# VitorMPCastro/MessyerRaytracer

Hardware: AMD Instinct MI355X
Metric: Mrays/s (primary, closest-hit) (higher is better)
Workload: dtype f32

## Files before the change

__graft_entry__.py:

```python
import os
import sys

ROOT = os.path.dirname(os.path.abspath(__file__))
if ROOT not in sys.path:
    sys.path.insert(0, ROOT)


def build() -> None:
    from messyerraytracer_amd import build as b
    b.build_lib()
    b.build_host_test()
    b.build_host_cpu_test()
    b.build_host_tlas_test()
    b.build_policy_test()
    b.build_shadow_policy_test()
    b.build_reflection_policy_test()
    b.build_hemisphere_policy_test()
    b.build_bounce_policy_test()
    b.build_instance_math_test()
    b.build_build_rules_test()
    b.build_shade_data_test()
    b.build_light_data_test()
    b.build_path_data_test()
    b.build_texture_data_test()
    b.build_panorama_data_test()
    b.build_channel_data_test()
    b.build_lane_map_test()
    from oracle import pyoracle
    pyoracle.build(force=False)
    if os.path.isdir("/root/reference") and not pyoracle.ref_available():
        pyoracle.build(force=True)
    import messyerraytracer_amd
    from messyerraytracer_amd import capi
    L = capi.load()
    missing = [s for s in capi.SYMBOLS if not hasattr(L, s)]
    if missing:
        raise RuntimeError(f"libmrt_hip.so does not export {missing}")


def smoke() -> None:
    import numpy as np
    from messyerraytracer_amd import capi, synth
    from oracle import pyoracle as po

    ctx = capi.Context(0)
    for verts, (w, h), origin, fwd, fov in (
            (synth.cube(), (16, 12), (0, 0, 3), (0, 0, -1), 60.0),
            (synth.soup(2000, 0.4, 3), (128, 96), (0, 0, -12), (0, 0, 1), 50.0)):
        scene = capi.Scene(verts)
        scene.upload(ctx)
        cam = capi.camera_look(origin, fwd, w, h, fov)
        got = ctx.cast_grid(cam, w, h)
        osc = po.OracleScene(verts)
        rays = po.grid_rays(origin, fwd, w, h, fov)
        want = osc.trace(rays)
        assert (got["prim_id"] == want["prim_id"]).all(), "prim_id mismatch vs oracle"
        hit = want["prim_id"] >= 0
        assert np.array_equal(got["t"][hit], want["t"][hit]), "t mismatch vs oracle"
        assert hit.any() and (~hit).any()
    local, inst = synth.multi_mesh_instances(4, 500, 0.3, 5)
    ctx.upload_two_level_scene(local, inst)
    got = ctx.cast_grid(cam, w, h)
    want = po.OracleTwoLevelScene(local, inst).trace(rays)
    assert (got["prim_id"] == want["prim_id"]).all() and np.array_equal(got["t"], want["t"]), "two-level scene mismatch vs oracle"
    assert (want["prim_id"] >= 0).any()
    from messyerraytracer_amd import surface as S, types as T
    n = w * h
    mats = np.zeros(2, T.MATERIAL)
    mats["albedo"], mats["roughness"], mats["emission"], mats["emission_energy"] = 0.5, (0.02, 0.7), 1.0, (0.0, 2.0)
    shade = S.ShadeData(1500, mats, np.arange(1500) % 3)
    ctx.upload_shade_data(shade.n_tris, shade.materials, shade.material_ids)
    d_hits, d_rows = ctx.device_alloc(n * 32), ctx.device_alloc(n * 64)
    ctx.h2d(d_hits, got)
    ctx.resolve_grid_surfaces(cam, w, h, d_hits, d_rows)
    rows = np.zeros(n, T.SURFACE64)
    ctx.d2h(rows, d_rows)
    surf, _, _ = S.resolve(rays["direction"], got["normal"], got["prim_id"] != -1, got["prim_id"].view(np.uint32), got["bary_u"],
                           got["bary_v"], shade)
    assert np.array_equal(rows.view(np.uint32), surf.view(np.uint32)), "surface rows mismatch vs the restatement"
    from messyerraytracer_amd import channels as Ch
    d_normal, d_depth8 = ctx.device_alloc(n * 16), ctx.device_alloc(n * 4)
    ctx.shade_grid_channels(cam, w, h, d_hits, 0.125, 1.0, {Ch.NORMAL: d_normal}, {Ch.DEPTH: d_depth8})
    normal, depth8 = np.zeros((n, 4), np.float32), np.zeros((n, 4), np.uint8)
    ctx.d2h(normal, d_normal)
    ctx.d2h(depth8, d_depth8)
    want = Ch.shade_channels(rays["direction"], Ch.hit_position(rays["origin"], rays["direction"], got["t"]), got["normal"],
                             got["prim_id"] != -1, got["t"], got["prim_id"].view(np.uint32), got["bary_u"], got["bary_v"],
                             np.float32(0.125), np.float32(1.0), shade, None, (Ch.NORMAL, Ch.DEPTH))
    assert np.array_equal(normal.view(np.uint32), want[Ch.NORMAL].view(np.uint32)), "normal channel mismatch vs the restatement"
    assert np.array_equal(depth8, Ch.to_rgba8(want[Ch.DEPTH])), "depth bytes mismatch vs the restatement"
    ctx.device_free(d_normal)
    ctx.device_free(d_depth8)
    ctx.device_free(d_hits)
    ctx.device_free(d_rows)
    ctx.close()
    print("smoke ok")


if __name__ == "__main__":
    build()
    if len(sys.argv) > 1 and sys.argv[1] == "smoke":
        smoke()
```

messyerraytracer_amd/build.py:

```python
import concurrent.futures
import glob
import os
import shutil
import subprocess

HERE = os.path.dirname(os.path.abspath(__file__))
CSRC = os.path.join(HERE, "csrc")
LIB = os.path.join(HERE, "libmrt_hip.so")
OBJ = os.path.join(HERE, "_obj")

SOURCES = ["kernels.hip", "shade_kernels.hip", "prep_kernels.hip", "api.hip", "cast.hip", "schedule.hip", "launch_policy.cpp", "group.hip",
           "device_build.hip", "refit.hip", "tlas_device.hip", "surface.hip", "texture.hip", "lighting.hip", "path.hip", "panorama.hip", "channels.hip",
           "host/shade_data.cpp", "host/texture_data.cpp", "host/light_data.cpp", "host/path_data.cpp", "host/panorama_data.cpp", "host/channel_data.cpp", "host/scene_prep.cpp", "host/bvh_builder.cpp", "host/two_level_prep.cpp"]
FLAGS = ["--offload-arch=gfx950", "-O3", "-std=c++17", "-fPIC", "-ffp-contract=off", "-Wall",
         "-Wno-unused-result", "-Xarch_host", "-mfma"]

MIRROR = ["-O2", "-std=c++17", "-ffp-contract=off", "-Wall"]
POLICY = ["-O2", "-std=c++17", "-Wall"]
CPU = ["-x", "c++", "-O2", "-std=c++17", "-ffp-contract=off", "-Wall"]
LANE = ["-x", "c++", "-std=c++17", "-Wall"]
DRIVERS = {
    "host_mirror_test": (["host/host_mirror_test.cpp"], MIRROR, True),
    "host_cpu_test": (["host/host_cpu_test.cpp"], MIRROR, True),
    "host_tlas_test": (["host/host_tlas_test.cpp"], MIRROR, True),
    "launch_policy_test": (["host/launch_policy_test.cpp", "launch_policy.cpp"], POLICY, False),
    "shadow_policy_test": (["host/shadow_policy_test.cpp", "launch_policy.cpp"], POLICY, False),
    "reflection_policy_test": (["host/reflection_policy_test.cpp", "launch_policy.cpp"], POLICY, False),
    "hemisphere_policy_test": (["host/hemisphere_policy_test.cpp", "launch_policy.cpp"], POLICY, False),
    "bounce_policy_test": (["host/bounce_policy_test.cpp", "launch_policy.cpp"], POLICY, False),
    "instance_math_test": (["host/instance_math_test.cpp"], CPU, False),
    "build_rules_test": (["host/build_rules_test.cpp"], CPU, False),
    "build_rules_test_san": (["host/build_rules_test.cpp"], CPU[:2] + ["-O1", "-g", "-fno-omit-frame-pointer", "-std=c++17", "-ffp-contract=off", "-Wall",
                                                               "-fsanitize=address,undefined", "-fno-sanitize-recover=undefined"], False),
    "shade_data_test": (["host/shade_data_test.cpp", "host/shade_data.cpp"], CPU, False),
    "light_data_test": (["host/light_data_test.cpp", "host/light_data.cpp"], CPU, False),
    "path_data_test": (["host/path_data_test.cpp", "host/path_data.cpp"], CPU, False),
    "texture_data_test": (["host/texture_data_test.cpp", "host/texture_data.cpp"], CPU, False),
    "panorama_data_test": (["host/panorama_data_test.cpp", "host/panorama_data.cpp"], CPU, False),
    "channel_data_test": (["host/channel_data_test.cpp", "host/channel_data.cpp"], CPU, False),
    "lane_map_test": (["host/lane_map_test.cpp"], LANE + ["-O2"], False),
    "lane_map_test_san": (["host/lane_map_test.cpp"], LANE + ["-O1", "-g", "-fno-omit-frame-pointer", "-fsanitize=address,undefined",
                                                              "-fno-sanitize-recover=undefined"], False),
}


def _hipcc() -> str:
    for c in (shutil.which("hipcc"), "/opt/rocm/bin/hipcc"):
        if c and os.path.exists(c):
            return c
    raise RuntimeError("hipcc not found: libmrt_hip.so cannot be built")


def _run(cmd, what: str) -> str:
    r = subprocess.run(cmd, capture_output=True, text=True, cwd=CSRC)
    if r.returncode != 0:
        raise RuntimeError(what + " failed:\n" + " ".join(cmd) + "\n" + r.stdout + r.stderr)
    return r.stderr


def _stale(target: str, deps) -> bool:
    if deps is None or not os.path.exists(target):
        return True
    t = os.path.getmtime(target)
    return any(not os.path.exists(d) or os.path.getmtime(d) > t for d in list(deps) + [os.path.abspath(__file__)])


def _deps(dfile: str):
    if not os.path.exists(dfile):
        return None
    with open(dfile) as f:
        words = f.read().replace("\\\n", " ").split()
    return [os.path.join(CSRC, w) for w in words if not w.endswith(":")]


def define_set(env) -> list:
    return sorted((["-DMRT_WITH_QUAD"] if env.get("MRT_WITH_QUAD") == "1" else []) + env.get("MRT_EXTRA_DEFINES", "").split())


def defines_changed(stamp, defines) -> bool:
    return stamp is None or stamp.split() != sorted(defines)


def pool_size(n_sources: int, env, limit: int = 16) -> int:
    jobs = min(n_sources, limit)
    if env.get("MAX_JOBS", "").isdigit() and int(env["MAX_JOBS"]) > 0:
        jobs = min(jobs, int(env["MAX_JOBS"]))
    return max(jobs, 1)


def build_lib(force: bool = False, verbose: bool = False, lib: str = None, obj_dir: str = None, defines=None) -> str:
    lib, obj_dir = os.path.abspath(lib or LIB), os.path.abspath(obj_dir or OBJ)
    defines = define_set(os.environ) if defines is None else sorted(defines)
    stamp = os.path.join(obj_dir, "defines.txt")
    objs = [os.path.join(obj_dir, s.replace("/", "_") + ".o") for s in SOURCES]
    old = open(stamp).read() if os.path.exists(stamp) else None
    force = force or defines_changed(old, defines)
    all_deps = [_deps(o + ".d") for o in objs]
    if not force and not _stale(lib, None if None in all_deps else [d for ds in all_deps for d in ds]):
        return lib
    os.makedirs(obj_dir, exist_ok=True)
    if force and old is not None:
        os.remove(stamp)
    jobs = [(s, o) for s, o, ds in zip(SOURCES, objs, all_deps) if force or _stale(o, ds)]

    def compile_one(job):
        src, obj = job
        log = _run([_hipcc()] + FLAGS + defines + ["-MD", "-MF", obj + ".d", "-c", os.path.join(CSRC, src), "-o", obj], "hipcc")
        with open(obj + ".d") as f:
            text = f.read().replace(CSRC + os.sep, "")
        with open(obj + ".d", "w") as f:
            f.write(text)
        return log

    with concurrent.futures.ThreadPoolExecutor(max_workers=pool_size(len(SOURCES), os.environ)) as pool:
        logs = list(pool.map(compile_one, jobs))
    with open(stamp, "w") as f:
        f.write(" ".join(defines) + "\n")
    if jobs or _stale(lib, objs):
        logs.append(_run([_hipcc(), "--offload-arch=gfx950", "-shared", "-fPIC"] + objs + ["-o", lib, "-pthread"], "hipcc link"))
    if verbose:
        print("".join(logs))
    return lib


def build_driver(name: str, force: bool = False) -> str:
    srcs, flags, links = DRIVERS[name]
    srcs, exe = [os.path.join(CSRC, s) for s in srcs], os.path.join(HERE, name)
    headers = [h for pat in ("*.h", "*.inc", "host/*.h", "host/*.hpp", "../../include/*.h") for h in glob.glob(os.path.join(CSRC, pat))]
    if force or _stale(exe, srcs + headers + ([LIB] if links else [])):
        _run([_hipcc()] + flags + srcs + ["-o", exe] + (["-L" + HERE, "-lmrt_hip", "-Wl,-rpath," + HERE, "-pthread"] if links else []), name + " build")
    return exe


def _driver(name: str):
    def build(force: bool = False) -> str:
        return build_driver(name, force)
    build.__doc__ = "C++ test driver " + name + " (DRIVERS)."
    return build


build_host_test = _driver("host_mirror_test")
build_host_cpu_test = _driver("host_cpu_test")
build_host_tlas_test = _driver("host_tlas_test")
build_policy_test = _driver("launch_policy_test")
build_shadow_policy_test = _driver("shadow_policy_test")
build_reflection_policy_test = _driver("reflection_policy_test")
build_hemisphere_policy_test = _driver("hemisphere_policy_test")
build_bounce_policy_test = _driver("bounce_policy_test")
build_instance_math_test = _driver("instance_math_test")
build_shade_data_test = _driver("shade_data_test")
build_light_data_test = _driver("light_data_test")
build_path_data_test = _driver("path_data_test")
build_texture_data_test = _driver("texture_data_test")
build_panorama_data_test = _driver("panorama_data_test")
build_channel_data_test = _driver("channel_data_test")


def build_build_rules_test(force: bool = False, sanitize: bool = False) -> str:
    return build_driver("build_rules_test_san" if sanitize else "build_rules_test", force)


def build_lane_map_test(force: bool = False, sanitize: bool = False) -> str:
    return build_driver("lane_map_test_san" if sanitize else "lane_map_test", force)


if __name__ == "__main__":
    print(build_lib(force=True, verbose=True))
    for name in DRIVERS:
        if not name.endswith("_san"):
            print(build_driver(name, force=True))
```

messyerraytracer_amd/csrc/kernels.hip:

```cpp
#include <hip/hip_runtime.h>
#include <cfloat>
#include <cstdio>
#include <cstdlib>
#include <type_traits>
#include "mrt_internal.h"
#include "launch_policy.h"
#include "lane_map.h"

namespace mrt {

#include "device_common.h"
#include "dispatch.h"

#include "source_common.h"
#include "shadow_kernel.h"
#include "reflection_kernel.h"
#include "hemisphere_kernel.h"
#include "bounce_kernel.h"

template <bool ANY_HIT, bool COUNT>
__global__ __launch_bounds__(MRT_WG) void trace_lane_kernel(const TraceParams p)
{
	constexpr int SRC = SRC_CAST;
	const NoSource s{};
#include "lane_walk.inc"
}

#include "lane_persistent_kernel.h"
#include "packet_kernel.h"
#include "packet_asm_kernel.h"
#include "packet_rows_kernel.h"
#ifdef MRT_WITH_QUAD
#include "packet_quad_kernel.h"
#endif
#include "two_level_kernel.h"

template <class S, int SRC, bool ANY_HIT>
__global__ __launch_bounds__(MRT_WG) void trace_source_lane_kernel(const TraceParams p, const S s)
{
	constexpr bool COUNT = false;
#include "lane_walk.inc"
}
template <class S, int SRC, bool ANY_HIT>
__global__ __launch_bounds__(MRT_WG) void trace_source_two_level_kernel(const TraceParams p, const S s)
{
#include "two_level_walk.inc"
}
template <class S, int SRC, bool ANY_HIT, int WIDTH, bool TL>
__global__ __launch_bounds__(MRT_WG) MRT_PERSIST_ATTR void trace_source_persistent_kernel(const TraceParams p, const PersistParams q, const S s)
{
	constexpr bool COUNT = false;
#include "persistent_walk.inc"
}

bool quad_kernel_built()
{
#ifdef MRT_WITH_QUAD
	return true;
#else
	return false;
#endif
}
static thread_local char g_variant[96] = "";
const char *last_trace_variant() { return g_variant; }
#ifndef MRT_ROWS_WG_LARGE
#define MRT_ROWS_WG_LARGE MRT_WG
#endif

hipError_t launch_trace(const TraceParams &p_in, bool any_hit, bool count, hipStream_t stream)
{
	const TraceLaunch l = resolve_trace(p_in, any_hit, count, quad_kernel_built(), MRT_ROWS_WG_LARGE);
	if (l.error) return hipErrorInvalidValue;
	if (l.blocks == 0) return hipSuccess;
	TraceParams p = p_in;
	p.tile_group = l.tile_group;
	const TraceVariant &v = l.v;
	const Bool a{v.any_hit}, c{v.count};
	const auto go = [&](auto kernel) { hipLaunchKernelGGL(kernel, dim3(l.blocks), dim3(l.threads), l.lds, stream, p); };
	switch (v.kernel) {
		case TraceKernel::TWO_LEVEL_PACKET: dispatch([&](auto A) { go(trace_two_level_packet_kernel<A>); }, a); break;
		case TraceKernel::TWO_LEVEL: dispatch([&](auto A) { go(trace_two_level_kernel<A>); }, a); break;
#ifdef MRT_WITH_QUAD
		case TraceKernel::PACKET_QUAD: dispatch([&](auto C, auto A) { go(trace_packet_quad_kernel<A, C>); }, c, a); break;
#endif
		case TraceKernel::PACKET_ROWS:
			if (v.packets == 2u)
				dispatch([&](auto W, auto F, auto C, auto A) { go(trace_packet_rows_kernel<A, C, 2, W, F>); },
						Among<64, MRT_ROWS_WG_LARGE>{(int)v.wg}, Bool{v.cull}, c, a);
			else dispatch([&](auto C, auto A) { go(trace_packet_rows_kernel<A, C, 1, MRT_WG, false>); }, c, a);
			break;
		case TraceKernel::PACKET_ASM:
			dispatch([&](auto C, auto KPF, auto A) { if constexpr (!(C && KPF)) go(trace_packet_asm_kernel<A, C, KPF>); }, c, Bool{v.prefetch}, a);
			break;
		case TraceKernel::PACKET: dispatch([&](auto A, auto C) { go(trace_packet_kernel<A, C>); }, a, c); break;
		case TraceKernel::LANE: dispatch([&](auto A, auto C) { go(trace_lane_kernel<A, C>); }, a, c); break;
		default: return hipErrorInvalidValue;
	}
	format_variant(g_variant, sizeof(g_variant), v);
	return hipGetLastError();
}

static PersistParams persist_params(const TraceParams &p, unsigned long long *next_ray, uint32_t *overflow,
		uint32_t lds_depth, uint32_t refill, uint32_t leaf_wait, uint32_t blocks)
{
	PersistParams q;
	q.next_ray = next_ray; q.overflow = overflow; q.overflow_stride = blocks * MRT_WG;
	q.lds_depth = lds_depth; q.refill = refill; q.leaf_wait = leaf_wait ? leaf_wait : 1u;
	const uint64_t per_wave = p.count / ((uint64_t)blocks * (MRT_WG / MRT_WAVE)) / 32u;
	q.chunk = per_wave >= MRT_RAY_CHUNK ? MRT_RAY_CHUNK : (per_wave <= MRT_WAVE ? MRT_WAVE : (uint32_t)(per_wave & ~63ull));
	return q;
}

hipError_t launch_trace_persistent(const TraceParams &p, unsigned long long *next_ray, uint32_t *overflow,
		uint32_t lds_depth, uint32_t refill, uint32_t leaf_wait, uint32_t blocks, bool any_hit, bool count, hipStream_t stream)
{
	const TraceLaunch l = resolve_persistent(p, lds_depth, blocks, any_hit, count);
	if (l.blocks == 0) return hipSuccess;
	const PersistParams q = persist_params(p, next_ray, overflow, lds_depth, refill, leaf_wait, blocks);
	const TraceVariant &v = l.v;
	dispatch([&](auto TL, auto C, auto W, auto A) {
		if constexpr (!TL || (W != 4 && !C))
			hipLaunchKernelGGL((trace_lane_persistent_kernel<A, W, TL, C>), dim3(l.blocks), dim3(l.threads), l.lds, stream, p, q);
	}, Bool{v.two_level}, Bool{v.count}, Among<8, 4, 2>{v.width}, Bool{v.any_hit});
	format_variant(g_variant, sizeof(g_variant), v);
	return hipGetLastError();
}

template <class S>
hipError_t launch_source(const TraceParams &p, const void *params, int src, bool any_hit, unsigned long long *next_ray, uint32_t *overflow,
		uint32_t lds_depth, uint32_t refill, uint32_t leaf_wait, uint32_t blocks, hipStream_t stream)
{
	using F = SourceFamily<S>;
	const S &s = *static_cast<const S *>(params);
	const TraceLaunch l = resolve_source(p, lds_depth, blocks, any_hit);
	if (l.error) return hipErrorInvalidValue;
	if (l.blocks == 0) return hipSuccess;
	if ((src != F::ray32 && src != F::host && src != F::grid) || !(any_hit ? F::any_hit : F::nearest)) return hipErrorInvalidValue;
	const TraceVariant &v = l.v;
	const dim3 grid(l.blocks), wg(l.threads);
	const PersistParams q = blocks ? persist_params(p, next_ray, overflow, lds_depth, refill, leaf_wait, blocks) : PersistParams{};
	dispatch([&](auto A, auto SRC, auto TL, auto W) {
		if constexpr ((A ? F::any_hit : F::nearest) && (!TL || W != 4)) {
			if (v.kernel == TraceKernel::TWO_LEVEL) hipLaunchKernelGGL((trace_source_two_level_kernel<S, SRC, A>), grid, wg, l.lds, stream, p, s);
			else if (v.kernel == TraceKernel::LANE) hipLaunchKernelGGL((trace_source_lane_kernel<S, SRC, A>), grid, wg, l.lds, stream, p, s);
			else hipLaunchKernelGGL((trace_source_persistent_kernel<S, SRC, A, W, TL>), grid, wg, l.lds, stream, p, q, s);
		}
	}, Bool{any_hit}, Among<F::ray32, F::host, F::grid>{src}, Bool{v.two_level}, Among<8, 4, 2>{v.width});
	format_variant(g_variant, sizeof(g_variant), v, F::name, src, F::any_hit && F::nearest);
	return hipGetLastError();
}
template hipError_t launch_source<ShadowParams>(const TraceParams &, const void *, int, bool, unsigned long long *, uint32_t *, uint32_t, uint32_t, uint32_t, uint32_t, hipStream_t);
template hipError_t launch_source<ReflectParams>(const TraceParams &, const void *, int, bool, unsigned long long *, uint32_t *, uint32_t, uint32_t, uint32_t, uint32_t, hipStream_t);
template hipError_t launch_source<HemiParams>(const TraceParams &, const void *, int, bool, unsigned long long *, uint32_t *, uint32_t, uint32_t, uint32_t, uint32_t, hipStream_t);
template hipError_t launch_source<BounceParams>(const TraceParams &, const void *, int, bool, unsigned long long *, uint32_t *, uint32_t, uint32_t, uint32_t, uint32_t, hipStream_t);

}
```

messyerraytracer_amd/csrc/lane_map.h:

```cpp
#pragma once
#include <cstdint>

#if defined(__HIPCC__) || defined(__HIP__)
#define MRT_LM_HD __host__ __device__ __forceinline__
#else
#define MRT_LM_HD inline
#endif

namespace mrt {

struct TileGrid {
	uint32_t grid_w, rows;
	uint32_t tiles_x, tiles_y;
	uint32_t k;
	uint32_t order;
	uint32_t group;
	uint32_t quarter_all;
	const uint32_t *sched;
	uint32_t unit, sched_slots;
};

constexpr uint32_t kPieceTile = 20u, kPieceTile16 = 21u, kPieceNone = 0xFFu;
constexpr uint32_t kNextAnew = 0u, kNextSame = 1u, kNextRight = 2u, kNextRowMajor = 3u, kNextNone = 4u;
struct WaveTile {
	uint32_t tx, ty;
	uint32_t code;
};

MRT_LM_HD uint32_t tile_rows_of(uint32_t rows, uint32_t k) { return (rows + (64u >> k) - 1u) >> (6u - k); }

MRT_LM_HD bool sched_matches(uint64_t total, uint32_t unit, uint32_t n_units)
{
	if (n_units == 0u) return total == 0u;
	return (uint64_t)(n_units - 1u) * unit < total && total <= (uint64_t)n_units * unit;
}

template <class T>
MRT_LM_HD bool strip_tile(const TileGrid &g, T tile, uint32_t &tx, uint32_t &ty)
{
	const uint32_t tg = g.group ? g.group : 1u;
	uint32_t m = (g.tiles_x + 128u) >> 8;
	if (m == 0u) m = 1u;
	const uint32_t S = g.tiles_x / (8u * m);
	if (S == 0u || S * 8u * m != g.tiles_x || S % tg != 0u) return false;
	const T wg = tile / tg;
	const uint32_t x = (uint32_t)wg & 7u;
	const T j = (wg >> 3) * tg + (tile - wg * tg);
	const T per_strip = (T)S * g.tiles_y;
	const T q = j / per_strip;
	const uint32_t sl = (uint32_t)q, r = (uint32_t)(j - q * per_strip);
	ty = r / S;
	tx = (sl * 8u + x) * S + r % S;
	return true;
}

template <class T>
MRT_LM_HD WaveTile wave_tile_t(const TileGrid &g, T group)
{
	WaveTile w; w.tx = 0u; w.ty = 0u; w.code = kPieceNone;
	const T total = (T)g.tiles_x * g.tiles_y;
	T tile = group;
	uint32_t piece = kPieceTile, next = kNextAnew;
	bool plus1 = false;
	if (g.quarter_all == 2u) {
		piece = (uint32_t)tile & 15u; tile >>= 4;
		if (tile >= total) return w;
		if (piece < 15u) next = kNextSame;
	} else if (g.quarter_all) {
		piece = 16u + ((uint32_t)tile & 3u); tile >>= 2;
		if (tile >= total) return w;
		if (piece < 19u) next = kNextSame;
	} else if (g.sched != nullptr) {
		const T slot = g.unit == 1u ? tile : (g.unit == 2u ? tile >> 1 : tile / g.unit);
		const uint32_t rem = (uint32_t)(tile - slot * g.unit);
		if (slot >= g.sched_slots) return w;
		const uint32_t e = g.sched[slot], what = e >> 28, id = e & 0x0FFFFFFFu;
		if (what == 0u) { tile = (T)id * g.unit + rem; plus1 = rem + 1u < g.unit; }
		else {
			if (rem != 0u) return w;
			tile = id;
			if (what >= 2u) piece = what - 2u < 4u ? 16u + (what - 2u) : kPieceTile16;
			if (g.unit > 1u) next = kNextNone;
		}
	} else plus1 = true;
	const bool even = ((uint32_t)tile & 1u) == 0u;
	if (g.order == 1u && (g.tiles_x & 15u) == 0u && (g.tiles_y & 15u) == 0u) {
		const uint32_t st = (uint32_t)(tile >> 8), in = (uint32_t)tile & 255u;
		uint32_t mx = in & 0x55u, my = (in >> 1) & 0x55u;
		mx = (mx | (mx >> 1)) & 0x33u; mx = (mx | (mx >> 2)) & 0x0Fu;
		my = (my | (my >> 1)) & 0x33u; my = (my | (my >> 2)) & 0x0Fu;
		const uint32_t sx = g.tiles_x >> 4, sty = st / sx;
		w.tx = ((st - sty * sx) << 4) + mx; w.ty = (sty << 4) + my;
		if (plus1 && even) next = kNextRight;
	} else if (g.order == 2u && (g.tiles_x & 31u) == 0u && (g.tiles_y & 31u) == 0u) {
		const uint32_t st = (uint32_t)(tile >> 10), in = (uint32_t)tile & 1023u;
		uint32_t mx = in & 0x155u, my = (in >> 1) & 0x155u;
		mx = (mx | (mx >> 1)) & 0x133u; mx = (mx | (mx >> 2)) & 0x10Fu; mx = (mx | (mx >> 4)) & 0x1Fu;
		my = (my | (my >> 1)) & 0x133u; my = (my | (my >> 2)) & 0x10Fu; my = (my | (my >> 4)) & 0x1Fu;
		const uint32_t sx = g.tiles_x >> 5, sty = st / sx;
		w.tx = ((st - sty * sx) << 5) + mx; w.ty = (sty << 5) + my;
		if (plus1 && even) next = kNextRight;
	} else if (g.order == 3u && strip_tile<T>(g, tile, w.tx, w.ty)) {
		if (plus1 && even && g.group != 0u && (g.group & 1u) == 0u) next = kNextRight;
	} else {
		const T y = tile / g.tiles_x;
		w.tx = (uint32_t)(tile - y * g.tiles_x); w.ty = (uint32_t)y;
		if (plus1) next = kNextRowMajor;
	}
	w.code = piece | next << 8;
	return w;
}

MRT_LM_HD WaveTile wave_tile(const TileGrid &g, uint64_t group)
{
	const bool narrow = (group >> 32) == 0u && (((uint64_t)g.tiles_x * g.tiles_y) >> 32) == 0u && (g.sched == nullptr || g.unit <= 16u);
	return narrow ? wave_tile_t<uint32_t>(g, (uint32_t)group) : wave_tile_t<uint64_t>(g, group);
}

MRT_LM_HD WaveTile wave_tile_next(const TileGrid &g, const WaveTile &a, uint64_t group)
{
	WaveTile b = a;
	const uint32_t piece = a.code & 0xFFu, next = piece == kPieceNone ? kNextAnew : a.code >> 8;
	b.code = piece | kNextAnew << 8;
	if (next == kNextSame) { b.code += 1u; return b; }
	if (next == kNextNone) { b.code = kPieceNone; return b; }
	if (next == kNextRight) { b.tx = a.tx + 1u; return b; }
	if (next == kNextRowMajor) {
		b.tx = a.tx + 1u;
		if (b.tx == g.tiles_x) { b.tx = 0u; b.ty = a.ty + 1u; }
		return b;
	}
	return wave_tile(g, group + 1u);
}

MRT_LM_HD bool tile_lane(const TileGrid &g, const WaveTile &w, uint32_t l, uint64_t &ray_idx, uint32_t &px, uint32_t &py)
{
	const uint32_t piece = w.code & 0xFFu;
	if (piece == kPieceNone) return false;
	if (piece < 16u) {
		if (l >= 4u) return false;
		px = (w.tx << 3) + ((piece & 3u) << 1) + (l & 1u);
		py = (w.ty << 3) + ((piece >> 2) << 1) + (l >> 1);
	} else if (piece < kPieceTile) {
		if (l >= 16u) return false;
		px = (w.tx << 3) + ((piece & 1u) << 2) + (l & 3u);
		py = (w.ty << 3) + (((piece >> 1) & 1u) << 2) + (l >> 2);
	} else {
		if (piece == kPieceTile16 && l >= 16u) return false;
		px = (w.tx << g.k) + (l & ((1u << g.k) - 1u));
		py = (w.ty << (6u - g.k)) + (l >> g.k);
	}
	if (px >= g.grid_w || py >= g.rows) return false;
	ray_idx = (uint64_t)py * g.grid_w + px;
	return true;
}

MRT_LM_HD bool linear_lane(uint64_t group, uint32_t l, uint32_t sparse_lanes, uint64_t count, uint64_t &entry)
{
	if (sparse_lanes) { if (l >= sparse_lanes) return false; entry = group * sparse_lanes + l; }
	else entry = (group << 6) + l;
	return entry < count;
}

}
```

messyerraytracer_amd/csrc/mrt_internal.h:

```cpp
#pragma once
#include <cstdint>
#include "../../include/mrt_hip.h"

static_assert(sizeof(mrt_ray32) == 32, "GPURayPacked must be 32 bytes (src/api/gpu_types.h:70)");
static_assert(sizeof(mrt_hit32) == 32, "GPUIntersectionPacked must be 32 bytes (src/api/gpu_types.h:93)");
static_assert(sizeof(mrt_tri64) == 64, "GPUTrianglePacked must be 64 bytes (src/api/gpu_types.h:51)");
static_assert(sizeof(mrt_bvh_node32) == 32, "GPUBVHNodePacked must be 32 bytes (src/api/gpu_types.h:127)");
static_assert(sizeof(mrt_bvh_node_wide64) == 64, "GPUBVHNodeWide must be 64 bytes (src/gpu/gpu_structs.h:47)");
static_assert(sizeof(mrt_host_ray60) == 60, "Ray must be 60 bytes (src/core/ray.h:25-51, precision=single)");
static_assert(sizeof(mrt_host_hit44) == 44, "Intersection must be 44 bytes (src/core/intersection.h:16-40)");
static_assert(sizeof(mrt_host_tri80) == 80, "Triangle must be 80 bytes (src/core/triangle.h:22-39)");
static_assert(sizeof(mrt_light) == 32, "mrt_light must be 32 bytes");

namespace mrt {

struct alignas(16) DevNode {
	float lmin[3]; uint32_t left_ref;
	float lmax[3]; uint32_t right_ref;
	float rmin[3]; uint32_t left_count;
	float rmax[3]; uint32_t right_count;
};
static_assert(sizeof(DevNode) == 64, "DevNode must be 64 bytes");

struct alignas(16) TriHot {
	float v0[3]; uint32_t id;
	float e1[3]; uint32_t layers;
	float e2[3]; uint32_t flags;
};
static_assert(sizeof(TriHot) == 48, "TriHot must be 48 bytes");
struct alignas(16) TriCold { float normal[3]; uint32_t pad; };

struct alignas(16) Dev4Node {
	float box[4][6];
	uint32_t ref[4];
	uint32_t n_children, pad[3];
};
static_assert(sizeof(Dev4Node) == 128, "Dev4Node must be 128 bytes");

struct alignas(16) Dev8Node {
	float org[3];
	uint8_t exp[3];
	uint8_t n_children;
	uint8_t qlo[3][8];
	uint8_t qhi[3][8];
	uint32_t ref[8];
	uint32_t pad[8];
};
static_assert(sizeof(Dev8Node) == 128, "Dev8Node must be 128 bytes");

constexpr int kCntRays = 0, kCntTris = 1, kCntNodes = 2, kCntHits = 3, kCntMaxStack = 4, kCntDeadPops = 5;
constexpr int kCntWaveNodeFetch = 6;
constexpr int kCntWaveTriFetch = 7;
constexpr int kCntLeafBoxChecks = 8;
constexpr int kCntFetchWaitCycles = 9, kCntWaveCycles = 10, kCntWaves = 11;
constexpr int kNumCounters = 16;
constexpr int kAutoGridOff = kNumCounters;
constexpr int kDetectScratchOff = kAutoGridOff + 8;
constexpr int kNextRayOff = kDetectScratchOff + 1026;
constexpr int kCounterWords = kNextRayOff + 128;

constexpr uint32_t kWaveSlots = 8192u;

constexpr uint32_t kSentinel = 0x7FFFFFFFu;
constexpr uint32_t kLeafBit = 0x80000000u;
constexpr uint32_t kLastInLeaf = 1u;

enum InFmt : uint32_t { IN_RAY32 = 0, IN_HOST60 = 1, IN_GRID = 2 };
enum OutFmt : uint32_t { OUT_HIT32 = 0, OUT_HOST44 = 1, OUT_BOOL8 = 2, OUT_TOKEN4 = 3, OUT_TOKEN8 = 4 };
enum LaneMap : uint32_t { MAP_LINEAR = 0, MAP_TILE8X8 = 1, MAP_AUTO = 2 };

struct DevInstance;
struct TraceParams {
	const DevNode *nodes;
	const Dev4Node *nodes4;
	const Dev8Node *nodes8;
	const float *leaf_box;
	const DevInstance *instances;
	const TriHot *tri_hot;
	const TriCold *tri_cold;
	const void *row_array;
	const void *row_array4;
	uint32_t rows_wg;
	uint32_t rows_cull;
	float scene_abs_max;
	uint32_t tri_unit_base4;
	const void *rays;
	void *hits;
	const uint32_t *perm;
	unsigned long long *counters;
	const uint32_t *auto_grid;
	const uint32_t *skip_flag;
	uint32_t skip_when;
	uint64_t count;
	uint32_t query_mask;
	uint32_t in_fmt, out_fmt, lane_map;
	uint32_t grid_w, grid_h, y0, rows;
	uint32_t tiles_x;
	uint32_t tile_w_log2;
	uint32_t tile_order;
	uint32_t tile_group;
	const uint32_t *tile_sched;
	uint32_t *tile_cost;
	uint32_t tile_unit, n_units;
	const uint32_t *sched_hdr;
	uint32_t n_slots_max;
	uint32_t quarter_all;
	uint32_t sparse_lanes;
	uint32_t kernel;
	uint32_t stack_depth;
	uint32_t xcd_swizzle;
	uint32_t n_tris;
	uint32_t n_instances;
	uint32_t n_nodes;
	uint32_t count_mode;
	uint32_t extra_lds;
	mrt_camera cam;
};

enum RaySrc : int { SRC_CAST = 0, SRC_SHADOW_RAY32 = 1, SRC_SHADOW_HOST44 = 2, SRC_SHADOW_GRID = 3,
	SRC_REFLECT_RAY32 = 4, SRC_REFLECT_HOST = 5, SRC_REFLECT_GRID = 6,
	SRC_HEMI_RAY32 = 7, SRC_HEMI_HOST = 8, SRC_HEMI_GRID = 9,
	SRC_BOUNCE_RAY32 = 10, SRC_BOUNCE_HOST = 11, SRC_BOUNCE_GRID = 12 };
constexpr bool shadow_source(int src) { return src >= SRC_SHADOW_RAY32 && src <= SRC_SHADOW_GRID; }
constexpr bool reflection_source(int src) { return src >= SRC_REFLECT_RAY32 && src <= SRC_REFLECT_GRID; }
constexpr bool hemisphere_source(int src) { return src >= SRC_HEMI_RAY32 && src <= SRC_HEMI_GRID; }
constexpr bool bounce_source(int src) { return src >= SRC_BOUNCE_RAY32 && src <= SRC_BOUNCE_GRID; }
constexpr bool lit_output(int src, bool any_hit) { return shadow_source(src) || (hemisphere_source(src) && any_hit); }
enum ShadowKind : uint32_t { SHADOW_OFF = 0, SHADOW_DIRECTIONAL = 1, SHADOW_POINT = 2 };
struct ShadowLight { uint32_t kind; float v[3]; };
struct ShadowParams {
	const void *records;
	uint64_t pixels;
	ShadowLight light[MRT_MAX_LIGHTS];
};

struct ReflectParams {
	const void *records;
	const uint8_t *select;
	void *out_rays;
	float max_distance;
};

constexpr uint32_t kPcgMul = 747796405u, kPcgInc = 2891336453u;
struct HemiJump { uint32_t a, c; };
struct HemiParams {
	const void *records;
	const uint8_t *select;
	void *out_rays;
	uint64_t pixels;
	uint32_t seed_add;
	float t_max;
	HemiJump jump[MRT_MAX_HEMISPHERE_SAMPLES];
};

struct BounceParams {
	const void *records;
	const uint8_t *select;
	const float *surface;
	void *out_rays;
	uint8_t *out_lobe;
	uint32_t seed_add;
	float t_max;
	float metallic, roughness;
	HemiJump jump;
};

enum SurfaceSrc : int { SURF_RAY32 = 0, SURF_HOST = 1, SURF_GRID = 2 };
struct SurfaceParams {
	const void *records;
	const void *shade_rows;
	const void *materials;
	uint32_t n_tris, n_materials, present;
	void *out_rows;
	float *out_bounce;
	void *out_hits;
};

struct ChannelParams {
	const void *records;
	const void *shade_rows;
	const void *materials;
	uint32_t n_tris, n_materials, present;
	uint32_t mask;
	float inv_depth_range, inv_pos_range;
	float *rgba[MRT_CHANNEL_COUNT];
	uint8_t *rgba8[MRT_CHANNEL_COUNT];
};
constexpr uint32_t CHANNELS_ROW = (1u << MRT_CHANNEL_NORMAL) | (1u << MRT_CHANNEL_ALBEDO) | (1u << MRT_CHANNEL_UV) | (1u << MRT_CHANNEL_FRESNEL);
constexpr uint32_t CHANNELS_MATERIAL = (1u << MRT_CHANNEL_NORMAL) | (1u << MRT_CHANNEL_ALBEDO);

template <class S> struct SourceFamily;
template <> struct SourceFamily<ShadowParams> {
	static constexpr int ray32 = SRC_SHADOW_RAY32, host = SRC_SHADOW_HOST44, grid = SRC_SHADOW_GRID;
	static constexpr bool any_hit = true, nearest = false;
	static constexpr const char *name = "shadow";
};
template <> struct SourceFamily<ReflectParams> {
	static constexpr int ray32 = SRC_REFLECT_RAY32, host = SRC_REFLECT_HOST, grid = SRC_REFLECT_GRID;
	static constexpr bool any_hit = false, nearest = true;
	static constexpr const char *name = "reflection";
};
template <> struct SourceFamily<HemiParams> {
	static constexpr int ray32 = SRC_HEMI_RAY32, host = SRC_HEMI_HOST, grid = SRC_HEMI_GRID;
	static constexpr bool any_hit = true, nearest = true;
	static constexpr const char *name = "hemisphere";
};
template <> struct SourceFamily<BounceParams> {
	static constexpr int ray32 = SRC_BOUNCE_RAY32, host = SRC_BOUNCE_HOST, grid = SRC_BOUNCE_GRID;
	static constexpr bool any_hit = false, nearest = true;
	static constexpr const char *name = "bounce";
};

struct DeviceSceneHost {
	DevNode *nodes = nullptr; uint32_t n_nodes = 0;
	Dev4Node *nodes4 = nullptr; uint32_t n_nodes4 = 0;
	uint32_t stack4 = 0;
	bool want8 = false;
	Dev8Node *nodes8 = nullptr; uint32_t n_nodes8 = 0; uint32_t stack8 = 0;
	float *leaf_box = nullptr;
	float bounds_lo[3] = {0, 0, 0}, bounds_hi[3] = {0, 0, 0};
	TriHot *hot = nullptr; TriCold *cold = nullptr; uint32_t n_tris = 0;
	uint32_t depth = 0;
};
int prepare_scene(const mrt_tri64 *tris, uint32_t n_tris, const mrt_bvh_node32 *nodes, uint32_t used_nodes,
		const uint32_t *prim_idx, DeviceSceneHost *out, char *err, size_t err_len);

struct DeviceBuildResult {
	DevNode *nodes = nullptr; TriHot *hot = nullptr; TriCold *cold = nullptr;
	Dev4Node *nodes4 = nullptr;
	Dev8Node *nodes8 = nullptr;
	float *leaf_box = nullptr;
	uint32_t n_nodes = 0, n_tris = 0, depth = 0, stack4 = 0, stack8 = 0;
	float bounds_lo[3] = {0, 0, 0}, bounds_hi[3] = {0, 0, 0};
	uint32_t *slot_src = nullptr;
	const float *boxes_in = nullptr;
};
struct BuildArena { void *ptr = nullptr; size_t cap = 0; uint32_t *pinned = nullptr; };
int device_build_lbvh(const mrt_tri64 *d_tris, uint32_t n, bool want4, bool want8, bool safe_handoff, int form, BuildArena *arena, void *stream,
		DeviceBuildResult *out, char *err, size_t err_len);

constexpr uint32_t kAsmNodeLimit = 1u << 26;
constexpr uint32_t kInstanceReturn = 0x7FFFFFFEu;
using ::MRT_KERNEL_TWO_LEVEL; using ::MRT_KERNEL_TWO_LEVEL_PACKET; using ::MRT_KERNEL_TWO_LEVEL_PERSISTENT;
using ::MRT_KERNEL_TWO_LEVEL_PERSISTENT8;
struct alignas(16) DevInstance {
	float inv[12];
	float basis[9];
	uint32_t root;
	uint32_t id_base;
	uint32_t layers;
	uint32_t flags;
	uint32_t index;
	uint32_t root8;
	uint32_t pad[5];
};
static_assert(sizeof(DevInstance) == 128, "DevInstance must be 128 bytes");

struct TwoLevelBlas { uint32_t first_tri, n_tris, root, depth; float lo[3], hi[3]; uint32_t root8, stack8, n_nodes; };
struct TwoLevelHost {
	DevNode *nodes = nullptr; uint32_t n_nodes = 0, tlas_cap = 0, n_tlas_nodes = 0;
	TriHot *hot = nullptr; TriCold *cold = nullptr; uint32_t n_tris = 0;
	DevInstance *inst = nullptr; uint32_t n_inst = 0;
	TwoLevelBlas *blas = nullptr; uint32_t n_blas = 0;
	uint32_t *inst_blas = nullptr;
	uint32_t depth = 0;
	Dev8Node *nodes8 = nullptr; uint32_t n_nodes8 = 0; float *leaf_box = nullptr;
	bool wide8 = false;
	uint32_t depth8 = 0;
	uint64_t flat_tris = 0;
};
void free_two_level(TwoLevelHost *h);
int prepare_two_level(const float *verts9, uint32_t n_mesh_tris, const mrt_instance *instances, uint32_t n_instances,
		uint32_t n_threads, bool build_blas, TwoLevelHost *out, char *err, size_t err_len);

int refit_two_level(TwoLevelHost *h, const mrt_instance *instances, uint32_t n_instances, char *err, size_t err_len);
int check_two_level_refit(const TwoLevelHost *h, const mrt_instance *instances, uint32_t n_instances, uint32_t n_mesh_tris,
		char *err, size_t err_len);

}
```

messyerraytracer_amd/csrc/packet_rows_kernel.h:

```cpp
#pragma once

#define RA_LMINX "s20"
#define RA_LMINY "s21"
#define RA_LMINZ "s22"
#define RA_LREF "s23"
#define RA_LMAXX "s24"
#define RA_LMAXY "s25"
#define RA_LMAXZ "s26"
#define RA_RREF "s27"
#define RA_RMINX "s28"
#define RA_RMINY "s29"
#define RA_RMINZ "s30"
#define RA_RMAXX "s32"
#define RA_RMAXY "s33"
#define RA_RMAXZ "s34"
#define RA_MASK "s[60:61]"
#define RA_MASKLO "s60"
#define RA_MASKHI "s61"
#define RA_V0X "s20"
#define RA_V0Y "s21"
#define RA_V0Z "s22"
#define RA_ID "s23"
#define RA_E1X "s24"
#define RA_E1Y "s25"
#define RA_E1Z "s26"
#define RA_LAYERS "s27"
#define RA_E2X "s28"
#define RA_E2Y "s29"
#define RA_E2Z "s30"
#define RA_FLAGS "s31"

#define MRT_NEAR_0(RS, AX, SIDE) RS##_##SIDE##MIN##AX
#define MRT_NEAR_1(RS, AX, SIDE) RS##_##SIDE##MAX##AX
#define MRT_FAR_0(RS, AX, SIDE) RS##_##SIDE##MAX##AX
#define MRT_FAR_1(RS, AX, SIDE) RS##_##SIDE##MIN##AX

#define MRT_OP(NAME, P) "%[" NAME P "]"

#define MRT_ROWS_SLAB(P, RS, BX, BY, BZ)                                                                             \
	"v_fma_f32 v50, " MRT_NEAR_##BX(RS, X, L) ", " MRT_OP("ix", P) ", " MRT_OP("nrx", P) "\n"                        \
	"v_fma_f32 v51, " MRT_NEAR_##BY(RS, Y, L) ", " MRT_OP("iy", P) ", " MRT_OP("nry", P) "\n"                        \
	"v_fma_f32 v52, " MRT_NEAR_##BZ(RS, Z, L) ", " MRT_OP("iz", P) ", " MRT_OP("nrz", P) "\n"                        \
	"v_fma_f32 v53, " MRT_FAR_##BX(RS, X, L) ", " MRT_OP("ix", P) ", " MRT_OP("nrx", P) "\n"                         \
	"v_fma_f32 v54, " MRT_FAR_##BY(RS, Y, L) ", " MRT_OP("iy", P) ", " MRT_OP("nry", P) "\n"                         \
	"v_fma_f32 v55, " MRT_FAR_##BZ(RS, Z, L) ", " MRT_OP("iz", P) ", " MRT_OP("nrz", P) "\n"                         \
	"v_max_f32 v52, v52, " MRT_OP("tmin", P) "\n"                                                                   \
	"v_fma_f32 v56, " MRT_NEAR_##BX(RS, X, R) ", " MRT_OP("ix", P) ", " MRT_OP("nrx", P) "\n"                        \
	"v_min_f32 v55, v55, " MRT_OP("lim", P) "\n"                                                                    \
	"v_fma_f32 v57, " MRT_NEAR_##BY(RS, Y, R) ", " MRT_OP("iy", P) ", " MRT_OP("nry", P) "\n"                        \
	"v_max3_f32 v50, v50, v51, v52\n"                                                               \
	"v_fma_f32 v51, " MRT_NEAR_##BZ(RS, Z, R) ", " MRT_OP("iz", P) ", " MRT_OP("nrz", P) "\n"                        \
	"v_min3_f32 v53, v53, v54, v55\n"                                                               \
	"v_fma_f32 v52, " MRT_FAR_##BX(RS, X, R) ", " MRT_OP("ix", P) ", " MRT_OP("nrx", P) "\n"                         \
	"v_fma_f32 v54, " MRT_FAR_##BY(RS, Y, R) ", " MRT_OP("iy", P) ", " MRT_OP("nry", P) "\n"                         \
	"v_fma_f32 v55, " MRT_FAR_##BZ(RS, Z, R) ", " MRT_OP("iz", P) ", " MRT_OP("nrz", P) "\n"                         \
	"v_max_f32 v51, v51, " MRT_OP("tmin", P) "\n"                                                                   \
	"v_min_f32 v55, v55, " MRT_OP("lim", P) "\n"                                                                    \
	"v_max3_f32 v56, v56, v57, v51\n"                                                               \
	"v_min3_f32 v52, v52, v54, v55\n"

#define MRT_ROWS_NODE_STEP(P, RS, POPBIT, CNT_P, BX, BY, BZ)                                                                 \
	MRT_ROWS_SLAB(P, RS, BX, BY, BZ)                                                                                \
	"v_cmp_le_f32 vcc, v50, v53\n"                                             \
	"v_cmp_le_f32_e64 s[54:55], v56, v52\n"                                    \
	"s_cbranch_vccz L_" P "lmiss_%=\n"                                                                              \
	"s_cmp_eq_u64 s[54:55], 0\n"                                                                                    \
	"s_cbranch_scc1 L_" P "onlyl_%=\n"                                                                              \
	"v_cmp_lt_f32_e64 s[56:57], v50, v56\n"     \
	"s_bitcmp1_b32 s56, 0\n"                                                                                        \
	"s_cselect_b32 s53, " RS##_RREF ", " RS##_LREF "\n"                                                    \
	"s_cselect_b32 " MRT_OP("cur", P) ", " RS##_LREF ", " RS##_RREF "\n"                                   \
	"s_cselect_b64 s[58:59], s[54:55], vcc\n"                                   \
	"s_cselect_b64 " RS##_MASK ", vcc, s[54:55]\n"                               \
	"v_mov_b32 v51, s53\n"                                                                                          \
	"v_mov_b32 v52, s58\n"                                                                                          \
	"v_mov_b32 v53, s59\n"                                                                                          \
	"ds_write_b32 " MRT_OP("sp", P) ", v51\n"                                                                       \
	"ds_write_b64 " MRT_OP("sp", P) ", v[52:53] offset:8\n"                                                         \
	"v_add_u32 " MRT_OP("sp", P) ", 16, " MRT_OP("sp", P) "\n"                                                      \
	CNT_P                                                                                                           \
	"v_lshlrev_b32 v54, 6, v51\n"             \
	"global_load_dword v60, v54, %[rows]\n"   \
	"s_branch L_" P "done_%=\n"                                                                                     \
	"L_" P "onlyl_%=:\n"                                                                                            \
	"s_mov_b32 " MRT_OP("cur", P) ", " RS##_LREF "\n"                                                                \
	"s_mov_b64 " RS##_MASK ", vcc\n"                                                                                 \
	"s_branch L_" P "done_%=\n"                                                                                     \
	"L_" P "lmiss_%=:\n"                                                                                            \
	"s_cmp_eq_u64 s[54:55], 0\n"                                                                                    \
	"s_cbranch_scc1 L_" P "npop_%=\n"                                                                               \
	"s_mov_b32 " MRT_OP("cur", P) ", " RS##_RREF "\n"                                                                \
	"s_mov_b64 " RS##_MASK ", s[54:55]\n"                                                                            \
	"s_branch L_" P "done_%=\n"                                                                                     \
	"L_" P "npop_%=:\n"                                                                                             \
	"s_or_b32 %[ev], %[ev], " POPBIT "\n"

#define MRT_ROWS_TRI_TEST(P, RS, OWNMASK, CUROP, ANYHIT_CODE)                                                        \
	"s_and_b32 s52, " RS##_LAYERS ", %[qmask]\n"                    \
	"s_cbranch_scc0 L_" P "tnext_%=\n"                                                                              \
	"v_mul_f32 v50, " RS##_E2Y ", " MRT_OP("dz", P) "\n"                                                             \
	"v_mul_f32 v51, " RS##_E2Z ", " MRT_OP("dx", P) "\n"                                                             \
	"v_mul_f32 v52, " RS##_E2X ", " MRT_OP("dy", P) "\n"                                                             \
	"v_fma_f32 v50, " MRT_OP("dy", P) ", " RS##_E2Z ", -v50\n"                            \
	"v_fma_f32 v51, " MRT_OP("dz", P) ", " RS##_E2X ", -v51\n"                            \
	"v_fma_f32 v52, " MRT_OP("dx", P) ", " RS##_E2Y ", -v52\n"                            \
	"v_mul_f32 v53, " RS##_E1Z ", v52\n"                                                                             \
	"v_fma_f32 v53, " RS##_E1Y ", v51, v53\n"                                                                        \
	"v_fma_f32 v53, " RS##_E1X ", v50, v53\n"                                                     \
	"v_cmp_nlt_f32_e64 s[54:55], |v53|, %[eps]\n"                                              \
	"s_and_b64 s[54:55], s[54:55], " OWNMASK "\n"                       \
	"s_cbranch_scc0 L_" P "tnext_%=\n"                                                                              \
	"v_div_scale_f32 v54, s[56:57], v53, v53, 1.0\n"                   \
	"v_rcp_f32 v55, v54\n"                                                                                          \
	"v_div_scale_f32 v56, vcc, 1.0, v53, 1.0\n"                                                                     \
	"v_subrev_f32 v59, " RS##_V0X ", " MRT_OP("ox", P) "\n"       \
	"v_fma_f32 v57, -v54, v55, 1.0\n"                                                                               \
	"v_fma_f32 v55, v57, v55, v55\n"                                                                                \
	"v_mul_f32 v57, v56, v55\n"                                                                                     \
	"v_fma_f32 v58, -v54, v57, v56\n"                                                                               \
	"v_fma_f32 v57, v58, v55, v57\n"                                                                                \
	"v_fma_f32 v54, -v54, v57, v56\n"                                                                               \
	"v_div_fmas_f32 v54, v54, v55, v57\n"                                                                           \
	"v_div_fixup_f32 v54, v54, v53, 1.0\n"                                                       \
	"v_subrev_f32 v55, " RS##_V0Y ", " MRT_OP("oy", P) "\n"                                                 \
	"v_subrev_f32 v56, " RS##_V0Z ", " MRT_OP("oz", P) "\n"                                                 \
	"v_mul_f32 v58, v56, v52\n"                                                                                     \
	"v_fma_f32 v58, v55, v51, v58\n"                                                                                \
	"v_fma_f32 v58, v59, v50, v58\n"                                                                                \
	"v_mul_f32 v58, v58, v54\n"                                                    \
	"v_cmp_nlt_f32_e64 s[56:57], v58, 0\n"                                                            \
	"v_cmp_ngt_f32_e64 s[58:59], v58, 1.0\n"                                                          \
	"s_and_b64 s[54:55], s[54:55], s[56:57]\n"                                                                      \
	"s_and_b64 s[54:55], s[54:55], s[58:59]\n"                                                                      \
	"s_cbranch_scc0 L_" P "tnext_%=\n"                                                                              \
	"v_mul_f32 v50, " RS##_E1Y ", v56\n"                                                                             \
	"v_mul_f32 v51, " RS##_E1Z ", v59\n"                                                                             \
	"v_mul_f32 v52, " RS##_E1X ", v55\n"                                                                             \
	"v_fma_f32 v50, v55, " RS##_E1Z ", -v50\n"                                          \
	"v_fma_f32 v51, v56, " RS##_E1X ", -v51\n"                                          \
	"v_fma_f32 v52, v59, " RS##_E1Y ", -v52\n"                                          \
	"v_mul_f32 v59, " MRT_OP("dz", P) ", v52\n"                                                                     \
	"v_fma_f32 v59, " MRT_OP("dy", P) ", v51, v59\n"                                                                \
	"v_fma_f32 v59, " MRT_OP("dx", P) ", v50, v59\n"                                                                \
	"v_mul_f32 v59, v59, v54\n"                                                     \
	"v_add_f32 v55, v58, v59\n"                                                                          \
	"v_cmp_nlt_f32_e64 s[56:57], v59, 0\n"                                                            \
	"v_cmp_ngt_f32_e64 s[58:59], v55, 1.0\n"                                                      \
	"s_and_b64 s[54:55], s[54:55], s[56:57]\n"                                                                      \
	"s_and_b64 s[54:55], s[54:55], s[58:59]\n"                                                                      \
	"s_cbranch_scc0 L_" P "tnext_%=\n"                                                                              \
	"v_mul_f32 v55, " RS##_E2Z ", v52\n"                                                                             \
	"v_fma_f32 v55, " RS##_E2Y ", v51, v55\n"                                                                        \
	"v_fma_f32 v55, " RS##_E2X ", v50, v55\n"                                                                        \
	"v_mul_f32 v55, v55, v54\n"                                                    \
	                          \
	"v_cmp_nlt_f32_e64 s[56:57], v55, " MRT_OP("tmin", P) "\n"                                                      \
	"v_cmp_lt_f32_e64 s[58:59], v55, " MRT_OP("lim", P) "\n"                                                        \
	"v_cmp_eq_f32_e64 s[64:65], v55, " MRT_OP("lim", P) "\n"                                                        \
	"v_cmp_ne_u32_e64 s[66:67], " MRT_OP("bs", P) ", -1\n"                                                          \
	"v_cmp_gt_u32_e64 vcc, " MRT_OP("bi", P) ", " RS##_ID "\n"                                     \
	"s_and_b64 s[64:65], s[64:65], s[66:67]\n"                                                                      \
	"s_and_b64 s[64:65], s[64:65], vcc\n"                                                                           \
	"s_or_b64 s[58:59], s[58:59], s[64:65]\n"                                                                       \
	"s_and_b64 s[54:55], s[54:55], s[56:57]\n"                                                                      \
	"s_and_b64 s[54:55], s[54:55], s[58:59]\n"                                    \
	"s_cbranch_scc0 L_" P "tnext_%=\n"                                                                              \
	"s_and_b32 s52, " CUROP ", 0x7fffffff\n"                                                \
	"v_mov_b32 v50, s52\n"                                                                                          \
	"v_mov_b32 v51, " RS##_ID "\n"                                                                                   \
	"v_cndmask_b32_e64 " MRT_OP("bt", P) ", " MRT_OP("bt", P) ", v55, s[54:55]\n"                                   \
	"v_cndmask_b32_e64 " MRT_OP("bu", P) ", " MRT_OP("bu", P) ", v58, s[54:55]\n"                                   \
	"v_cndmask_b32_e64 " MRT_OP("bv", P) ", " MRT_OP("bv", P) ", v59, s[54:55]\n"                                   \
	"v_cndmask_b32_e64 " MRT_OP("bs", P) ", " MRT_OP("bs", P) ", v50, s[54:55]\n"                                   \
	"v_cndmask_b32_e64 " MRT_OP("bi", P) ", " MRT_OP("bi", P) ", v51, s[54:55]\n"                                   \
	ANYHIT_CODE                                                                                                     \
	"L_" P "tnext_%=:\n"

#define MRT_ROWS_TRI_STEP(P, RS, POPBIT, CNT_T, ANYHIT_CODE)                                                         \
	CNT_T                                                                                                           \
	MRT_ROWS_TRI_TEST(P, RS, RS##_MASK, MRT_OP("cur", P), ANYHIT_CODE)                                              \
	"s_bitcmp1_b32 " RS##_FLAGS ", 0\n"                                          \
	"s_cbranch_scc1 L_" P "tpop_%=\n"                                                                               \
	"s_add_u32 " MRT_OP("cur", P) ", " MRT_OP("cur", P) ", 1\n"                                                     \
	"s_branch L_" P "done_%=\n"                                                                                     \
	"L_" P "tpop_%=:\n"                                                                                             \
	"s_or_b32 %[ev], %[ev], " POPBIT "\n"

#define MRT_ROWS_NEAREST(P) \
	"v_cndmask_b32_e64 " MRT_OP("lim", P) ", " MRT_OP("lim", P) ", v55, s[54:55]\n"
#define MRT_ROWS_ANYHIT(P, DONEBIT) \
	"v_cndmask_b32_e64 " MRT_OP("lim", P) ", " MRT_OP("lim", P) ", %[vneg], s[54:55]\n"                             \
	"v_cmp_neq_f32_e64 s[56:57], " MRT_OP("lim", P) ", %[vneg]\n"                                                   \
	"s_cmp_lg_u64 s[56:57], 0\n"                                                                                    \
	"s_cbranch_scc1 L_" P "tnext_%=\n"                                                                              \
	"s_mov_b32 " MRT_OP("cur", P) ", 0x7fffffff\n"                                                                  \
	"s_or_b32 %[ev], %[ev], " DONEBIT "\n"                                                                          \
	"s_branch L_" P "done_%=\n"

#define MRT_ROWS_STEP(P, RS, POPBIT, CNT_N, CNT_T, CNT_P, ANYHIT_CODE, BX, BY, BZ)                                            \
	"s_bitcmp1_b32 " MRT_OP("cur", P) ", 31\n"                                                                      \
	"s_cbranch_scc1 L_" P "tri_%=\n"                                                                                \
	CNT_N                                                                                                           \
	MRT_ROWS_NODE_STEP(P, RS, POPBIT, CNT_P, BX, BY, BZ)                                                             \
	"s_branch L_" P "done_%=\n"                                                                                     \
	"L_" P "tri_%=:\n"                                                                                              \
	MRT_ROWS_TRI_STEP(P, RS, POPBIT, CNT_T, ANYHIT_CODE)                                                             \
	"L_" P "done_%=:\n"

#define MRT_ROWS_POP_ISSUE(P, POPBITNO, V0123)                                                                      \
	"s_bitcmp1_b32 %[ev], " POPBITNO "\n"                                                                           \
	"s_cbranch_scc0 L_" P "pi_%=\n"                                                                                 \
	"v_add_u32 " MRT_OP("sp", P) ", -16, " MRT_OP("sp", P) "\n"                                                     \
	"ds_read_b128 " V0123 ", " MRT_OP("sp", P) "\n"                                                                 \
	"L_" P "pi_%=:\n"
#define MRT_ROWS_POP_TAKE(P, RS, POPBITNO, V0, V2, V3)                                                               \
	"s_bitcmp1_b32 %[ev], " POPBITNO "\n"                                                                           \
	"s_cbranch_scc0 L_" P "pt_%=\n"                                                                                 \
	"v_readfirstlane_b32 " MRT_OP("cur", P) ", " V0 "\n"                                                            \
	"v_readfirstlane_b32 " RS##_MASKLO ", " V2 "\n"                                                                  \
	"v_readfirstlane_b32 " RS##_MASKHI ", " V3 "\n"                                                                  \
	"L_" P "pt_%=:\n"

#define MRT_ROWS_CLOBBERS                                                                                             \
	"vcc", "scc", "s20", "s21", "s22", "s23", "s24", "s25", "s26", "s27", "s28", "s29", "s30", "s31", "s32", "s33", \
	"s34", "s35", "s36", "s37", "s38", "s39", "s40", "s41", "s42", "s43", "s44", "s45", "s46", "s47", "s48", "s49", \
	"s50", "s51", "s52", "s53", "s54", "s55", "s56", "s57", "s58", "s59", "s60", "s61", "s62", "s63", "s64", "s65", \
	"s66", "s67", "v50", "v51", "v52", "v53", "v54", "v55", "v56", "v57", "v58", "v59", "v60"

#define MRT_ROWS_OUT(P, S)                                                                                            \
	[cur##P] "+s"(S.cur), [sp##P] "+v"(S.sp), [lim##P] "+v"(S.lim), [bt##P] "+v"(S.bt), [bu##P] "+v"(S.bu),         \
	[bv##P] "+v"(S.bv), [bs##P] "+v"(S.bs), [bi##P] "+v"(S.bi), [mask##P] "+s"(S.mask)
#define MRT_ROWS_IN(P, S)                                                                                             \
	[ox##P] "v"(S.ox), [oy##P] "v"(S.oy), [oz##P] "v"(S.oz), [dx##P] "v"(S.dx), [dy##P] "v"(S.dy), [dz##P] "v"(S.dz), \
	[tmin##P] "v"(S.tmin), [ix##P] "v"(S.ix), [iy##P] "v"(S.iy), [iz##P] "v"(S.iz), [nrx##P] "v"(S.nrx),            \
	[nry##P] "v"(S.nry), [nrz##P] "v"(S.nrz)

struct PacketRegs {
	float ox, oy, oz, dx, dy, dz, tmin;
	float ix, iy, iz, nrx, nry, nrz;
	float lim;
	float bt, bu, bv;
	uint32_t bs, bi;
	uint32_t sp;
	uint32_t cur;
	unsigned long long mask;
};

#define MRT_ROWS_LOOP1(CNT_N, CNT_T, CNT_P, T_PRE, T_POST, ANYHIT_CODE, BX, BY, BZ)                                          \
	asm volatile(                                                                                                   \
		"s_mov_b64 s[60:61], %[maskA]\n"                                                                            \
		"L_loop_%=:\n"                                                                                              \
		"s_lshl_b32 s52, %[curA], 6\n"                                                                              \
		T_PRE                                                                                                       \
		"s_load_dwordx16 s[20:35], %[rows], s52\n"                                                                  \
		"s_waitcnt lgkmcnt(0)\n"                                                                                    \
		T_POST                                                                                                      \
		MRT_ROWS_STEP("A", RA, "1", CNT_N, CNT_T, CNT_P, ANYHIT_CODE, BX, BY, BZ)                                   \
		"s_cmp_eq_u32 %[ev], 0\n"                                                                                   \
		"s_cbranch_scc1 L_loop_%=\n"                                                                                \
		MRT_ROWS_POP_ISSUE("A", "0", "v[50:53]")                                                                    \
		"s_waitcnt lgkmcnt(0)\n"                                                                                    \
		MRT_ROWS_POP_TAKE("A", RA, "0", "v50", "v52", "v53")                                                        \
		"s_mov_b32 %[ev], 0\n"                                                                                      \
		"s_cmp_lg_u32 %[curA], 0x7fffffff\n"                                                                        \
		"s_cbranch_scc1 L_loop_%=\n"                                                                                \
		"s_waitcnt vmcnt(0)\n"                    \
		"s_mov_b64 %[maskA], s[60:61]\n"                                                                            \
		: MRT_ROWS_OUT(A, a), [ev] "+s"(ev), [cntn] "+s"(cnt_n), [cntt] "+s"(cnt_t), [cntw] "+s"(cnt_w), [cntp] "+s"(sp_max) \
		: MRT_ROWS_IN(A, a), [rows] "s"(rows), [qmask] "s"(qmask), [eps] "s"(eps), [vneg] "v"(vneg)                 \
		: MRT_ROWS_CLOBBERS)

#define MRT_ROWSW_GROUP_SLAB(P, OWN, LM, RM, BX, BY, BZ)                                                              \
	"s_cmp_eq_u64 " OWN ", 0\n"                                                                                     \
	"s_cbranch_scc1 L_" P "skip_%=\n"                             \
	MRT_ROWS_SLAB(P, RA, BX, BY, BZ)                                                                                \
	"v_cmp_le_f32_e64 " LM ", v50, v53\n"                                                                           \
	"v_cmp_le_f32_e64 " RM ", v56, v52\n"                                                                           \
	"L_" P "sdone_%=:\n"
#define MRT_ROWSW_GROUP_SKIP(P, LM, RM)                                                                               \
	"L_" P "skip_%=:\n"                                                                                             \
	"s_mov_b64 " LM ", 0\n"                                                                                         \
	"s_mov_b64 " RM ", 0\n"                                                                                         \
	"s_branch L_" P "sdone_%=\n"

#define MRT_ROWSW_ANYHIT(P) \
	"v_cndmask_b32_e64 " MRT_OP("lim", P) ", " MRT_OP("lim", P) ", %[vneg], s[54:55]\n"
#define MRT_ROWSW_ANYDONE                                                                                             \
	"v_cmp_neq_f32_e64 s[56:57], %[limA], %[vneg]\n"                                                                \
	"v_cmp_neq_f32_e64 s[58:59], %[limB], %[vneg]\n"                                                                \
	"s_or_b64 s[56:57], s[56:57], s[58:59]\n"                                                                       \
	"s_cbranch_scc1 L_goon_%=\n"                                                                                    \
	"s_mov_b32 %[curA], 0x7fffffff\n"                                                                               \
	"s_branch L_exit_%=\n"                                                                                          \
	"L_goon_%=:\n"

#ifndef MRT_ROWS_KPREFETCH
#define MRT_ROWS_KPREFETCH 1
#endif
#if MRT_ROWS_KPREFETCH
#define MRT_ROWSW_KPREFETCH                                                                                           \
	"s_lshl_b32 s48, " RA_LREF ", 6\n"                                                                               \
	"s_lshl_b32 s49, " RA_RREF ", 6\n"                                                                               \
	"s_load_dword s64, %[rows], s48\n"                                                                              \
	"s_load_dword s65, %[rows], s49\n"
#define MRT_ROWSW_FARPREFETCH ""
#else
#define MRT_ROWSW_KPREFETCH ""
#define MRT_ROWSW_FARPREFETCH                                                                                         \
	"v_lshlrev_b32 v55, 6, v54\n"                                       \
	"global_load_dword v60, v55, %[rows]\n"
#endif

#define MRT_ROWS_LOOPW(CNT_N, CNT_T, CNT_P, ANYA, ANYB, ANYDONE, BX, BY, BZ)                                                 \
	asm volatile(                                                                                                   \
		"s_mov_b64 s[60:61], %[maskA]\n"                                                                            \
		"s_mov_b64 s[62:63], %[maskB]\n"                                                                            \
		"L_loop_%=:\n"                                                                                              \
		"s_lshl_b32 s52, %[curA], 6\n"                                                                              \
		"s_load_dwordx16 s[20:35], %[rows], s52\n"                                                                  \
		"s_waitcnt lgkmcnt(0)\n"                                                                                    \
		"s_bitcmp1_b32 %[curA], 31\n"                                                                               \
		"s_cbranch_scc1 L_tri_%=\n"                                                                                 \
		CNT_N                                                                                                       \
		MRT_ROWSW_KPREFETCH                                                                                         \
		MRT_ROWSW_GROUP_SLAB("A", "s[60:61]", "s[36:37]", "s[38:39]", BX, BY, BZ)                                   \
		MRT_ROWSW_GROUP_SLAB("B", "s[62:63]", "s[40:41]", "s[42:43]", BX, BY, BZ)                                   \
		"s_or_b64 s[44:45], s[36:37], s[40:41]\n"                     \
		"s_cbranch_scc0 L_lmiss_%=\n"                                                                               \
		"s_or_b64 vcc, s[38:39], s[42:43]\n"                                              \
		"s_cbranch_scc0 L_onlyl_%=\n"                                                                               \
		      \
		"v_cmp_lt_f32_e64 s[46:47], v50, v56\n"                                           \
		"s_bitcmp1_b32 s46, 0\n"                                                                                    \
		"s_cselect_b32 s53, " RA_RREF ", " RA_LREF "\n"                                                   \
		"s_cselect_b32 %[curA], " RA_LREF ", " RA_RREF "\n"                                               \
		"s_cselect_b64 s[50:51], s[38:39], s[36:37]\n"                 \
		"s_cselect_b64 s[58:59], s[42:43], s[40:41]\n"                                                              \
		"s_cselect_b64 s[60:61], s[36:37], s[38:39]\n"                                        \
		"s_cselect_b64 s[62:63], s[40:41], s[42:43]\n"                                                              \
		"v_mov_b32 v50, s50\n"                                                                                      \
		"v_mov_b32 v51, s51\n"                                                                                      \
		"v_mov_b32 v52, s58\n"                                                                                      \
		"v_mov_b32 v53, s59\n"                                                                                      \
		"v_mov_b32 v54, s53\n"                                                                                      \
		"ds_write_b128 %[spA], v[50:53]\n"                                                                          \
		"ds_write_b32 %[spA], v54 offset:16\n"                                                                      \
		"v_add_u32 %[spA], 32, %[spA]\n"                                                                            \
		CNT_P                                                                                                       \
		MRT_ROWSW_FARPREFETCH                                                                                       \
		"s_branch L_loop_%=\n"                                                                                      \
		"L_onlyl_%=:\n"                                                                                             \
		"s_mov_b32 %[curA], " RA_LREF "\n"                                                                          \
		"s_mov_b64 s[60:61], s[36:37]\n"                                                                            \
		"s_mov_b64 s[62:63], s[40:41]\n"                                                                            \
		"s_branch L_loop_%=\n"                                                                                      \
		"L_lmiss_%=:\n"                                                                                             \
		"s_or_b64 vcc, s[38:39], s[42:43]\n"                                                                        \
		"s_cbranch_scc0 L_pop_%=\n"                                                                                 \
		"s_mov_b32 %[curA], " RA_RREF "\n"                                                                          \
		"s_mov_b64 s[60:61], s[38:39]\n"                                                                            \
		"s_mov_b64 s[62:63], s[42:43]\n"                                                                            \
		"s_branch L_loop_%=\n"                                                                                      \
		"L_tri_%=:\n"                                                                                               \
		CNT_T                                                                                                       \
		"s_cmp_eq_u64 s[60:61], 0\n"                                                                                \
		"s_cbranch_scc1 L_Atnext_%=\n"                                                                              \
		MRT_ROWS_TRI_TEST("A", RA, "s[60:61]", "%[curA]", ANYA)                                                     \
		"s_cmp_eq_u64 s[62:63], 0\n"                                                                                \
		"s_cbranch_scc1 L_Btnext_%=\n"                                                                              \
		MRT_ROWS_TRI_TEST("B", RA, "s[62:63]", "%[curA]", ANYB)                                                     \
		ANYDONE                                                                                                     \
		"s_bitcmp1_b32 " RA_FLAGS ", 0\n"                                       \
		"s_cbranch_scc1 L_pop_%=\n"                                                                                 \
		"s_add_u32 %[curA], %[curA], 1\n"                                                                           \
		"s_branch L_loop_%=\n"                                                                                      \
		"L_pop_%=:\n"                                                                                               \
		"v_add_u32 %[spA], -32, %[spA]\n"                                                                           \
		"ds_read_b128 v[50:53], %[spA]\n"                                                                           \
		"ds_read_b32 v54, %[spA] offset:16\n"                                                                       \
		"s_waitcnt lgkmcnt(0)\n"                                                                                    \
		"v_readfirstlane_b32 %[curA], v54\n"                                                                        \
		"v_readfirstlane_b32 s60, v50\n"                                                                            \
		"v_readfirstlane_b32 s61, v51\n"                                                                            \
		"v_readfirstlane_b32 s62, v52\n"                                                                            \
		"v_readfirstlane_b32 s63, v53\n"                                                                            \
		"s_cmp_lg_u32 %[curA], 0x7fffffff\n"                                                                        \
		"s_cbranch_scc1 L_loop_%=\n"                                                                                \
		"s_branch L_exit_%=\n"                                                                                      \
		MRT_ROWSW_GROUP_SKIP("A", "s[36:37]", "s[38:39]")                                                           \
		MRT_ROWSW_GROUP_SKIP("B", "s[40:41]", "s[42:43]")                                                           \
		"L_exit_%=:\n"                                                                                              \
		"s_waitcnt vmcnt(0)\n"                    \
		"s_mov_b64 %[maskA], s[60:61]\n"                                                                            \
		"s_mov_b64 %[maskB], s[62:63]\n"                                                                            \
		: MRT_ROWS_OUT(A, a), [limB] "+v"(b.lim), [btB] "+v"(b.bt), [buB] "+v"(b.bu), [bvB] "+v"(b.bv),             \
		  [bsB] "+v"(b.bs), [biB] "+v"(b.bi), [maskB] "+s"(b.mask), [cntn] "+s"(cnt_n), [cntt] "+s"(cnt_t), [cntp] "+s"(sp_max) \
		: MRT_ROWS_IN(A, a), MRT_ROWS_IN(B, b), [rows] "s"(rows), [qmask] "s"(qmask), [eps] "s"(eps), [vneg] "v"(vneg) \
		: MRT_ROWS_CLOBBERS)


#define MRT_ROWS_SLAB1(P, RS, SIDE, TE, BX, BY, BZ, MASK)                                                             \
	"v_fma_f32 v51, " MRT_NEAR_##BX(RS, X, SIDE) ", " MRT_OP("ix", P) ", " MRT_OP("nrx", P) "\n"                      \
	"v_fma_f32 v52, " MRT_NEAR_##BY(RS, Y, SIDE) ", " MRT_OP("iy", P) ", " MRT_OP("nry", P) "\n"                      \
	"v_fma_f32 v53, " MRT_NEAR_##BZ(RS, Z, SIDE) ", " MRT_OP("iz", P) ", " MRT_OP("nrz", P) "\n"                      \
	"v_fma_f32 v54, " MRT_FAR_##BX(RS, X, SIDE) ", " MRT_OP("ix", P) ", " MRT_OP("nrx", P) "\n"                       \
	"v_fma_f32 v55, " MRT_FAR_##BY(RS, Y, SIDE) ", " MRT_OP("iy", P) ", " MRT_OP("nry", P) "\n"                       \
	"v_fma_f32 v57, " MRT_FAR_##BZ(RS, Z, SIDE) ", " MRT_OP("iz", P) ", " MRT_OP("nrz", P) "\n"                       \
	"v_max_f32 v53, v53, " MRT_OP("tmin", P) "\n"                                                                   \
	"v_min_f32 v57, v57, " MRT_OP("lim", P) "\n"                                                                    \
	"v_max3_f32 " TE ", v51, v52, v53\n"                                                                            \
	"v_min3_f32 v54, v54, v55, v57\n"                                                                               \
	"v_cmp_le_f32_e64 " MASK ", " TE ", v54\n"

#define MRT_ROWSC_CHILD(SIDE, TE, CULLBITS, MA, MB, BX, BY, BZ)                                                       \
	"s_and_b32 s48, s44, " CULLBITS "\n"                                 \
	"s_cbranch_scc1 L_cull" #SIDE "_%=\n"                                                                           \
	"s_cmp_eq_u64 s[60:61], 0\n"                                                                                    \
	"s_cbranch_scc1 L_" #SIDE "A0_%=\n"                                                                             \
	MRT_ROWS_SLAB1("A", RA, SIDE, TE, BX, BY, BZ, MA)                                                               \
	"L_" #SIDE "A1_%=:\n"                                                                                           \
	"s_cmp_eq_u64 s[62:63], 0\n"                                                                                    \
	"s_cbranch_scc1 L_" #SIDE "B0_%=\n"                                                                             \
	MRT_ROWS_SLAB1("B", RA, SIDE, TE, BX, BY, BZ, MB)                                                               \
	"L_" #SIDE "B1_%=:\n"
#define MRT_ROWSC_CHILD_OOL(SIDE, MA, MB)                                                                             \
	"L_cull" #SIDE "_%=:\n"                                                                                         \
	MRT_ROWSC_CNT_CULL                                                                                              \
	"s_mov_b64 " MA ", 0\n"                                                                                         \
	"s_mov_b64 " MB ", 0\n"                                                                                         \
	"s_branch L_" #SIDE "B1_%=\n"                                                                                   \
	"L_" #SIDE "A0_%=:\n"                                                                                           \
	"s_mov_b64 " MA ", 0\n"                                                                                         \
	"s_branch L_" #SIDE "A1_%=\n"                                                                                   \
	"L_" #SIDE "B0_%=:\n"                                                                                           \
	"s_mov_b64 " MB ", 0\n"                                                                                         \
	"s_branch L_" #SIDE "B1_%=\n"
#define MRT_ROWSC_CNT_CULL ""

#define MRT_ROWSC_VLOAD(VDST, REF)                                                                                   \
	"v_lshl_add_u32 v62, " REF ", 6, %[cvo]\n"                                                                      \
	"global_load_dword " VDST ", v62, %[rows]\n"

#ifndef MRT_ROWSC_KPF
#define MRT_ROWSC_KPF 0
#endif
#if MRT_ROWSC_KPF
#define MRT_ROWSC_KPREFETCH                                                                                           \
	"s_lshl_b32 s46, " RA_LREF ", 6\n"                                                                               \
	"s_lshl_b32 s47, " RA_RREF ", 6\n"                                                                               \
	"s_load_dword s64, %[rows], s46\n"                                                                              \
	"s_load_dword s65, %[rows], s47\n"
#else
#define MRT_ROWSC_KPREFETCH ""
#endif
#define MRT_ROWS_LOOPC(CNT_N, CNT_T, CNT_P, ANYA, ANYB, ANYDONE, BX, BY, BZ)                                          \
	asm volatile(                                                                                                   \
		"s_mov_b64 s[60:61], %[maskA]\n"                                                                            \
		"s_mov_b64 s[62:63], %[maskB]\n"                                                                            \
		"L_vload_%=:\n"                                     \
		MRT_ROWSC_VLOAD("v60", "%[curA]")                                                                           \
		"s_mov_b64 s[66:67], 0\n"                                                                                   \
		"L_loop_%=:\n"                                                                                              \
		"s_lshl_b32 s52, %[curA], 6\n"                                                                              \
		"s_load_dwordx16 s[20:35], %[rows], s52\n"                                                                  \
		"s_waitcnt lgkmcnt(0)\n"                                                                                    \
		"s_bitcmp1_b32 %[curA], 31\n"                                                                               \
		"s_cbranch_scc1 L_tri_%=\n"                                                                                 \
		CNT_N                                                                                                       \
		"s_waitcnt vmcnt(0)\n"                      \
		"v_cndmask_b32_e64 v58, v60, v61, s[66:67]\n"                                                               \
		"v_mul_f32 v58, v58, %[cw]\n"                                                                               \
		MRT_ROWSC_VLOAD("v60", RA_LREF)            \
		"v_add_f32_dpp v59, v58, v58 row_shr:1 row_mask:0xf bank_mask:0xf bound_ctrl:1\n"  \
		MRT_ROWSC_VLOAD("v61", RA_RREF)                                                                             \
		"v_add_f32_dpp v58, v59, v59 row_shr:2 row_mask:0xf bank_mask:0xf bound_ctrl:1\n"                           \
		"s_nop 1\n"                                                                                                 \
		"v_add_f32_dpp v59, v58, v58 row_shr:4 row_mask:0xf bank_mask:0xf bound_ctrl:1\n"                           \
		"v_cmp_lt_f32_e64 s[44:45], v59, %[ccc]\n"  \
		MRT_ROWSC_KPREFETCH                                                                                         \
		"s_or_b32 s44, s44, s45\n"                                                                                  \
		MRT_ROWSC_CHILD(L, "v50", "0x00800080", "s[36:37]", "s[40:41]", BX, BY, BZ)                                 \
		MRT_ROWSC_CHILD(R, "v56", "0x80008000", "s[38:39]", "s[42:43]", BX, BY, BZ)                                 \
		"s_or_b64 s[44:45], s[36:37], s[40:41]\n"                     \
		"s_cbranch_scc0 L_lmiss_%=\n"                                                                               \
		"s_or_b64 vcc, s[38:39], s[42:43]\n"                                              \
		"s_cbranch_scc0 L_onlyl_%=\n"                                                                               \
		      \
		"v_cmp_lt_f32_e64 s[46:47], v50, v56\n"                                           \
		"s_bitcmp1_b32 s46, 0\n"                                                                                    \
		"s_cselect_b32 s53, " RA_RREF ", " RA_LREF "\n"                                                   \
		"s_cselect_b32 %[curA], " RA_LREF ", " RA_RREF "\n"                                               \
		"s_cselect_b64 s[50:51], s[38:39], s[36:37]\n"                 \
		"s_cselect_b64 s[58:59], s[42:43], s[40:41]\n"                                                              \
		"s_cselect_b64 s[60:61], s[36:37], s[38:39]\n"                                        \
		"s_cselect_b64 s[62:63], s[40:41], s[42:43]\n"                                                              \
		"s_cselect_b64 s[66:67], 0, -1\n"                       \
		"v_mov_b32 v50, s50\n"                                                                                      \
		"v_mov_b32 v51, s51\n"                                                                                      \
		"v_mov_b32 v52, s58\n"                                                                                      \
		"v_mov_b32 v53, s59\n"                                                                                      \
		"v_mov_b32 v54, s53\n"                                                                                      \
		"ds_write_b128 %[spA], v[50:53]\n"                                                                          \
		"ds_write_b32 %[spA], v54 offset:16\n"                                                                      \
		"v_add_u32 %[spA], 32, %[spA]\n"                                                                            \
		CNT_P                                                                                                       \
		"s_branch L_loop_%=\n"                                                                                      \
		"L_onlyl_%=:\n"                                                                                             \
		"s_mov_b32 %[curA], " RA_LREF "\n"                                                                          \
		"s_mov_b64 s[60:61], s[36:37]\n"                                                                            \
		"s_mov_b64 s[62:63], s[40:41]\n"                                                                            \
		"s_mov_b64 s[66:67], 0\n"                                                                                   \
		"s_branch L_loop_%=\n"                                                                                      \
		"L_lmiss_%=:\n"                                                                                             \
		"s_or_b64 vcc, s[38:39], s[42:43]\n"                                                                        \
		"s_cbranch_scc0 L_pop_%=\n"                                                                                 \
		"s_mov_b32 %[curA], " RA_RREF "\n"                                                                          \
		"s_mov_b64 s[60:61], s[38:39]\n"                                                                            \
		"s_mov_b64 s[62:63], s[42:43]\n"                                                                            \
		"s_mov_b64 s[66:67], -1\n"                                                                                  \
		"s_branch L_loop_%=\n"                                                                                      \
		"L_tri_%=:\n"                                                                                               \
		CNT_T                                                                                                       \
		"s_cmp_eq_u64 s[60:61], 0\n"                                                                                \
		"s_cbranch_scc1 L_Atnext_%=\n"                                                                              \
		MRT_ROWS_TRI_TEST("A", RA, "s[60:61]", "%[curA]", ANYA)                                                     \
		"s_cmp_eq_u64 s[62:63], 0\n"                                                                                \
		"s_cbranch_scc1 L_Btnext_%=\n"                                                                              \
		MRT_ROWS_TRI_TEST("B", RA, "s[62:63]", "%[curA]", ANYB)                                                     \
		ANYDONE                                                                                                     \
		"s_bitcmp1_b32 " RA_FLAGS ", 0\n"                                       \
		"s_cbranch_scc1 L_pop_%=\n"                                                                                 \
		"s_add_u32 %[curA], %[curA], 1\n"                                                                           \
		"s_branch L_loop_%=\n"                                                                                      \
		"L_pop_%=:\n"                                                                                               \
		"v_add_u32 %[spA], -32, %[spA]\n"                                                                           \
		"ds_read_b128 v[50:53], %[spA]\n"                                                                           \
		"ds_read_b32 v54, %[spA] offset:16\n"                                                                       \
		"s_waitcnt lgkmcnt(0)\n"                                                                                    \
		"v_readfirstlane_b32 %[curA], v54\n"                                                                        \
		"v_readfirstlane_b32 s60, v50\n"                                                                            \
		"v_readfirstlane_b32 s61, v51\n"                                                                            \
		"v_readfirstlane_b32 s62, v52\n"                                                                            \
		"v_readfirstlane_b32 s63, v53\n"                                                                            \
		"s_cmp_lg_u32 %[curA], 0x7fffffff\n"                                                                        \
		"s_cbranch_scc1 L_vload_%=\n"                                                                               \
		"s_branch L_exit_%=\n"                                                                                      \
		MRT_ROWSC_CHILD_OOL(L, "s[36:37]", "s[40:41]")                                                              \
		MRT_ROWSC_CHILD_OOL(R, "s[38:39]", "s[42:43]")                                                              \
		"L_exit_%=:\n"                                                                                              \
		"s_waitcnt vmcnt(0)\n"                 \
		"s_mov_b64 %[maskA], s[60:61]\n"                                                                            \
		"s_mov_b64 %[maskB], s[62:63]\n"                                                                            \
		: MRT_ROWS_OUT(A, a), [limB] "+v"(b.lim), [btB] "+v"(b.bt), [buB] "+v"(b.bu), [bvB] "+v"(b.bv),             \
		  [bsB] "+v"(b.bs), [biB] "+v"(b.bi), [maskB] "+s"(b.mask), [cntn] "+s"(cnt_n), [cntt] "+s"(cnt_t), [cntp] "+s"(sp_max) \
		: MRT_ROWS_IN(A, a), MRT_ROWS_IN(B, b), [rows] "s"(rows), [qmask] "s"(qmask),                                \
		  [eps] "s"(eps), [vneg] "v"(vneg), [cw] "v"(cull.w), [ccc] "v"(cull.cc), [cvo] "v"(cull.voff)               \
		: MRT_ROWS_CLOBBERS, "v61", "v62")

struct CullRegs {
	float w;
	float cc;
	uint32_t voff;
};

#define MRT_ROWS_T_PRE "s_memtime s[64:65]\n s_waitcnt lgkmcnt(0)\n"
#define MRT_ROWS_T_POST "s_memtime s[66:67]\n s_waitcnt lgkmcnt(0)\n s_sub_u32 s64, s66, s64\n s_add_u32 %[cntw], %[cntw], s64\n"
#define MRT_ROWS_CNT_N "s_add_u32 %[cntn], %[cntn], 1\n"
#define MRT_ROWS_CNT_P "v_readfirstlane_b32 s52, %[spA]\n s_max_u32 %[cntp], %[cntp], s52\n"
#define MRT_ROWS_CNT_T "s_add_u32 %[cntt], %[cntt], 1\n"

__device__ __forceinline__ void rows_uniform(PacketRegs &s)
{
	s.cur = __builtin_amdgcn_readfirstlane(s.cur);
	const uint32_t lo = __builtin_amdgcn_readfirstlane((uint32_t)s.mask), hi = __builtin_amdgcn_readfirstlane((uint32_t)(s.mask >> 32));
	s.mask = ((unsigned long long)hi << 32) | lo;
}

template <int OCT, bool ANY_HIT, bool COUNT>
__device__ __forceinline__ void rows_walk_one(const float4 *rows, uint32_t qmask, PacketRegs &a, uint32_t &cnt_n, uint32_t &cnt_t, uint32_t &cnt_w, uint32_t &sp_max)
{
	const float eps = 1e-8f, vneg = -FLT_MAX;
	uint32_t ev = 0u;
#define MRT_W1(O, BX, BY, BZ)                                                                                         \
	if (OCT == O) {                                                                                                 \
		if (COUNT) { if (ANY_HIT) MRT_ROWS_LOOP1(MRT_ROWS_CNT_N, MRT_ROWS_CNT_T, MRT_ROWS_CNT_P, MRT_ROWS_T_PRE, MRT_ROWS_T_POST, MRT_ROWS_ANYHIT("A", "4"), BX, BY, BZ); \
			else MRT_ROWS_LOOP1(MRT_ROWS_CNT_N, MRT_ROWS_CNT_T, MRT_ROWS_CNT_P, MRT_ROWS_T_PRE, MRT_ROWS_T_POST, MRT_ROWS_NEAREST("A"), BX, BY, BZ); } \
		else { if (ANY_HIT) MRT_ROWS_LOOP1("", "", "", "", "", MRT_ROWS_ANYHIT("A", "4"), BX, BY, BZ);              \
			else MRT_ROWS_LOOP1("", "", "", "", "", MRT_ROWS_NEAREST("A"), BX, BY, BZ); }                           \
	}
	MRT_W1(0, 0, 0, 0) MRT_W1(1, 1, 0, 0) MRT_W1(2, 0, 1, 0) MRT_W1(3, 1, 1, 0) MRT_W1(4, 0, 0, 1) MRT_W1(5, 1, 0, 1) MRT_W1(6, 0, 1, 1) MRT_W1(7, 1, 1, 1)
#undef MRT_W1
	rows_uniform(a);
	cnt_n = __builtin_amdgcn_readfirstlane(cnt_n); cnt_t = __builtin_amdgcn_readfirstlane(cnt_t); cnt_w = __builtin_amdgcn_readfirstlane(cnt_w);
	sp_max = __builtin_amdgcn_readfirstlane(sp_max);
}

template <int OCT, bool ANY_HIT, bool COUNT>
__device__ __forceinline__ void rows_walk_wide(const float4 *rows, uint32_t qmask, PacketRegs &a, PacketRegs &b, uint32_t &cnt_n, uint32_t &cnt_t, uint32_t &sp_max)
{
	const float eps = 1e-8f, vneg = -FLT_MAX;
#define MRT_WW(O, BX, BY, BZ)                                                                                         \
	if (OCT == O) {                                                                                                 \
		if (COUNT) { if (ANY_HIT) MRT_ROWS_LOOPW(MRT_ROWS_CNT_N, MRT_ROWS_CNT_T, MRT_ROWS_CNT_P, MRT_ROWSW_ANYHIT("A"), MRT_ROWSW_ANYHIT("B"), MRT_ROWSW_ANYDONE, BX, BY, BZ); \
			else MRT_ROWS_LOOPW(MRT_ROWS_CNT_N, MRT_ROWS_CNT_T, MRT_ROWS_CNT_P, MRT_ROWS_NEAREST("A"), MRT_ROWS_NEAREST("B"), "", BX, BY, BZ); } \
		else { if (ANY_HIT) MRT_ROWS_LOOPW("", "", "", MRT_ROWSW_ANYHIT("A"), MRT_ROWSW_ANYHIT("B"), MRT_ROWSW_ANYDONE, BX, BY, BZ); \
			else MRT_ROWS_LOOPW("", "", "", MRT_ROWS_NEAREST("A"), MRT_ROWS_NEAREST("B"), "", BX, BY, BZ); }        \
	}
	MRT_WW(0, 0, 0, 0) MRT_WW(1, 1, 0, 0) MRT_WW(2, 0, 1, 0) MRT_WW(3, 1, 1, 0) MRT_WW(4, 0, 0, 1) MRT_WW(5, 1, 0, 1) MRT_WW(6, 0, 1, 1) MRT_WW(7, 1, 1, 1)
#undef MRT_WW
	rows_uniform(a);
	cnt_n = __builtin_amdgcn_readfirstlane(cnt_n); cnt_t = __builtin_amdgcn_readfirstlane(cnt_t);
	sp_max = __builtin_amdgcn_readfirstlane(sp_max);
}

template <int OCT, bool ANY_HIT, bool COUNT>
__device__ __forceinline__ void rows_walk_cull(const float4 *rows, uint32_t qmask, PacketRegs &a, PacketRegs &b, const CullRegs &cull, uint32_t &cnt_n, uint32_t &cnt_t, uint32_t &sp_max)
{
	const float eps = 1e-8f, vneg = -FLT_MAX;
#define MRT_WC(O, BX, BY, BZ)                                                                                         \
	if (OCT == O) {                                                                                                 \
		if (COUNT) { if (ANY_HIT) MRT_ROWS_LOOPC(MRT_ROWS_CNT_N, MRT_ROWS_CNT_T, MRT_ROWS_CNT_P, MRT_ROWSW_ANYHIT("A"), MRT_ROWSW_ANYHIT("B"), MRT_ROWSW_ANYDONE, BX, BY, BZ); \
			else MRT_ROWS_LOOPC(MRT_ROWS_CNT_N, MRT_ROWS_CNT_T, MRT_ROWS_CNT_P, MRT_ROWS_NEAREST("A"), MRT_ROWS_NEAREST("B"), "", BX, BY, BZ); } \
		else { if (ANY_HIT) MRT_ROWS_LOOPC("", "", "", MRT_ROWSW_ANYHIT("A"), MRT_ROWSW_ANYHIT("B"), MRT_ROWSW_ANYDONE, BX, BY, BZ); \
			else MRT_ROWS_LOOPC("", "", "", MRT_ROWS_NEAREST("A"), MRT_ROWS_NEAREST("B"), "", BX, BY, BZ); }        \
	}
	MRT_WC(0, 0, 0, 0) MRT_WC(1, 1, 0, 0) MRT_WC(2, 0, 1, 0) MRT_WC(3, 1, 1, 0) MRT_WC(4, 0, 0, 1) MRT_WC(5, 1, 0, 1) MRT_WC(6, 0, 1, 1) MRT_WC(7, 1, 1, 1)
#undef MRT_WC
	rows_uniform(a);
	cnt_n = __builtin_amdgcn_readfirstlane(cnt_n); cnt_t = __builtin_amdgcn_readfirstlane(cnt_t);
	sp_max = __builtin_amdgcn_readfirstlane(sp_max);
}

__device__ __forceinline__ CullRegs cull_setup(const RayRegs &ra, const RayRegs &rb, bool valid_a, bool valid_b, unsigned long long part_a,
		unsigned long long part_b, float scene_abs_max, uint32_t lane)
{
	CullRegs c;
	c.w = 0.0f; c.cc = -__builtin_inff(); c.voff = (lane & 15u) * 4u;
	const bool corners = (part_a & 1ull) && (part_a >> 56 & 1ull) && (part_b >> 7 & 1ull) && (part_b >> 63 & 1ull);
	if (!corners) return c;
#define MRT_RL(v, l) __builtin_bit_cast(float, __builtin_amdgcn_readlane(__builtin_bit_cast(int, v), l))
	const float ox = MRT_RL(ra.ox, 0), oy = MRT_RL(ra.oy, 0), oz = MRT_RL(ra.oz, 0);
	const float tl[3] = { MRT_RL(ra.dx, 0), MRT_RL(ra.dy, 0), MRT_RL(ra.dz, 0) }, bl[3] = { MRT_RL(ra.dx, 56), MRT_RL(ra.dy, 56), MRT_RL(ra.dz, 56) };
	const float tr[3] = { MRT_RL(rb.dx, 7), MRT_RL(rb.dy, 7), MRT_RL(rb.dz, 7) }, br[3] = { MRT_RL(rb.dx, 63), MRT_RL(rb.dy, 63), MRT_RL(rb.dz, 63) };
	float cen[3] = { tl[0] + tr[0] + bl[0] + br[0], tl[1] + tr[1] + bl[1] + br[1], tl[2] + tr[2] + bl[2] + br[2] };
	const float cl = __builtin_sqrtf(cen[0] * cen[0] + cen[1] * cen[1] + cen[2] * cen[2]);
	if (!(cl > 0.0f)) return c;
	cen[0] /= cl; cen[1] /= cl; cen[2] /= cl;
	const uint32_t k = lane >> 4;
	const float *pa = k == 0u ? tl : (k == 1u ? tr : (k == 2u ? br : bl)), *pb = k == 0u ? tr : (k == 1u ? br : (k == 2u ? bl : tl));
	float n[3] = { pa[1] * pb[2] - pa[2] * pb[1], pa[2] * pb[0] - pa[0] * pb[2], pa[0] * pb[1] - pa[1] * pb[0] };
	const float nl = __builtin_sqrtf(n[0] * n[0] + n[1] * n[1] + n[2] * n[2]);
	bool ok = nl > 0.0f;
	const float inv = ok ? 1.0f / nl : 0.0f;
	n[0] *= inv; n[1] *= inv; n[2] *= inv;
	if (n[0] * cen[0] + n[1] * cen[1] + n[2] * cen[2] < 0.0f) { n[0] = -n[0]; n[1] = -n[1]; n[2] = -n[2]; }
	const float push = 5e-5f;
	n[0] += push * cen[0]; n[1] += push * cen[1]; n[2] += push * cen[2];
	bool inside = true;
	for (int q = 0; q < 4; q++) {
		const float qx = MRT_RL(n[0], 16 * q), qy = MRT_RL(n[1], 16 * q), qz = MRT_RL(n[2], 16 * q);
		const float da = qx * ra.dx + qy * ra.dy + qz * ra.dz, la = __builtin_sqrtf(ra.dx * ra.dx + ra.dy * ra.dy + ra.dz * ra.dz);
		const float db = qx * rb.dx + qy * rb.dy + qz * rb.dz, lb = __builtin_sqrtf(rb.dx * rb.dx + rb.dy * rb.dy + rb.dz * rb.dz);
		if (valid_a && !(da >= 1e-5f * la)) inside = false;
		if (valid_b && !(db >= 1e-5f * lb)) inside = false;
	}
#undef MRT_RL
	if (valid_a && !(ra.ox == ox && ra.oy == oy && ra.oz == oz && ra.t_min >= 0.0f)) inside = false;
	if (valid_b && !(rb.ox == ox && rb.oy == oy && rb.oz == oz && rb.t_min >= 0.0f)) inside = false;
	ok = ok && __builtin_isfinite(n[0]) && __builtin_isfinite(n[1]) && __builtin_isfinite(n[2]);
	const bool planes_ok = (__ballot(ok) & 0x0001000100010001ull) == 0x0001000100010001ull;
	if (__ballot(!inside) != 0ull || !planes_ok) return c;
	const float n1 = __builtin_fabsf(n[0]) + __builtin_fabsf(n[1]) + __builtin_fabsf(n[2]);
	const float o1 = __builtin_fabsf(ox) + __builtin_fabsf(oy) + __builtin_fabsf(oz);
	const float err = 8.0f * 5.9604645e-8f * n1 * (scene_abs_max + o1);
	const float cc = (n[0] * ox + n[1] * oy + n[2] * oz) - err;
	if (__ballot(!__builtin_isfinite(cc)) != 0ull) return c;
	const uint32_t d = lane & 15u, axis = d & 3u;
	const bool is_max = (d >> 2 & 1u) != 0u;
	const float na = axis == 0u ? n[0] : (axis == 1u ? n[1] : n[2]);
	c.w = (axis < 3u && ((na >= 0.0f) == is_max)) ? na : 0.0f;
	c.cc = (d == 7u || d == 15u) ? cc : -__builtin_inff();
	return c;
}

__device__ __forceinline__ void rows_init(PacketRegs &s, const RayRegs &r, bool takes_part, uint32_t sp)
{
	s.ox = r.ox; s.oy = r.oy; s.oz = r.oz; s.dx = r.dx; s.dy = r.dy; s.dz = r.dz; s.tmin = r.t_min;
	s.ix = safe_inv(r.dx); s.iy = safe_inv(r.dy); s.iz = safe_inv(r.dz);
	s.nrx = -(r.ox * s.ix); s.nry = -(r.oy * s.iy); s.nrz = -(r.oz * s.iz);
	s.bt = r.t_max; s.bu = 0.0f; s.bv = 0.0f; s.bs = 0xFFFFFFFFu; s.bi = 0xFFFFFFFFu;
	s.lim = (!takes_part || r.t_min >= r.t_max) ? -FLT_MAX : r.t_max;
	s.sp = sp; s.cur = 0u; s.mask = 0ull;
}

__device__ __forceinline__ int rows_octant(const RayRegs &r, bool part, unsigned long long &part_mask)
{
	part_mask = __ballot(part);
	const unsigned long long sx = __ballot(part && safe_inv(r.dx) < 0.0f), sy = __ballot(part && safe_inv(r.dy) < 0.0f),
			sz = __ballot(part && safe_inv(r.dz) < 0.0f);
	const bool uniform = (sx == 0ull || sx == part_mask) && (sy == 0ull || sy == part_mask) && (sz == 0ull || sz == part_mask);
	return uniform ? ((sx ? 1 : 0) | (sy ? 2 : 0) | (sz ? 4 : 0)) : 8;
}

__device__ __forceinline__ void rows_hit_of_slot(const float4 *rows, uint32_t n_nodes, uint32_t slot, PacketRegs &s)
{
	s.bs = 0xFFFFFFFFu;
	if (slot != 0xFFFFFFFFu) { s.bs = slot + n_nodes; s.bi = __float_as_uint(rows[(size_t)s.bs * 4u].w); }
}

template <bool STREAM>
__device__ __forceinline__ void finish_row_ray(const TraceParams &p, const float4 *rows, uint64_t ray_idx, const RayRegs &r,
		float best_t, float best_u, float best_v, uint32_t best_row, uint32_t best_id, uint32_t best_slot)
{
	int32_t prim = -1; float nx = 0.0f, ny = 0.0f, nz = 0.0f; uint32_t layers = 0u;
	if (best_row != 0xFFFFFFFFu) {
		if (p.out_fmt == OUT_BOOL8 || p.out_fmt == OUT_TOKEN4) prim = 0;
		else {
			const float4 *row = rows + (size_t)best_row * 4u;
			prim = (int32_t)best_id;
			layers = __float_as_uint(reinterpret_cast<const float *>(row)[7]);
			const float4 nn = row[3];
			nx = nn.x; ny = nn.y; nz = nn.z;
		}
	}
	store_hit<STREAM>(p, ray_idx, r, best_t, prim, best_u, best_v, nx, ny, nz, layers, best_slot);
}

#ifndef MRT_ROWS_WPE
#define MRT_ROWS_WPE 8
#endif
template <bool ANY_HIT, bool COUNT, int PACKETS, int WG, bool CULL = false>
__global__ __launch_bounds__(WG) __attribute__((amdgpu_waves_per_eu(MRT_ROWS_WPE, 8))) void trace_packet_rows_kernel(const TraceParams p)
{
	__shared__ __attribute__((aligned(16))) uint32_t wave_stack[WG / MRT_WAVE][PACKETS][(MRT_PACKET_STACK + 1) * 4];
	if (skip_launch(p)) return;
	constexpr bool STREAM = WG == MRT_WAVE;
	uint32_t block = blockIdx.x;
	if (p.xcd_swizzle) {
		const uint32_t per = gridDim.x >> 3;
		if (block < (per << 3)) block = (block & 7u) * per + (block >> 3);
	}
	const uint32_t wave = threadIdx.x / MRT_WAVE, lane = threadIdx.x & (MRT_WAVE - 1);
	const uint32_t wave_s = __builtin_amdgcn_readfirstlane(wave), block_s = block;
	const uint64_t group_a = ((uint64_t)block_s * (WG / MRT_WAVE) + wave_s) * PACKETS;
	TileGrid tg;
	const bool tiled = tile_grid(p, tg);
	WaveTile ta = {0u, 0u, kPieceNone}, tb = ta;
	if (tiled) {
		ta = wave_tile(tg, group_a);
		if (PACKETS == 2) tb = wave_tile_next(tg, ta, group_a);
	}
	const uint32_t tile_ax = __builtin_amdgcn_readfirstlane(ta.tx), tile_ay = __builtin_amdgcn_readfirstlane(ta.ty);
	const uint32_t tile_bx = __builtin_amdgcn_readfirstlane(tb.tx), tile_by = __builtin_amdgcn_readfirstlane(tb.ty);
	const uint32_t tile_code = __builtin_amdgcn_readfirstlane((ta.code & 0xFFu) | (tb.code & 0xFFu) << 8 | (tiled ? 1u << 16 : 0u));
	uint64_t idx = 0; uint32_t px = 0, py = 0;
	const bool valid_a = tiled ? tile_lane(tg, ta, lane, idx, px, py) : linear_ray(p, group_a, lane, idx, px, py);
	RayRegs ra = {0.0f, 0.0f, 0.0f, 0.0f, 0.0f, 0.0f, 1.0f, 0.0f}, rb = ra;
	if (valid_a) load_ray<STREAM>(p, idx, px, py, ra);
	bool valid_b = false;
	if (PACKETS == 2) {
		valid_b = tiled ? tile_lane(tg, tb, lane, idx, px, py) : linear_ray(p, group_a + 1u, lane, idx, px, py);
		if (valid_b) load_ray<STREAM>(p, idx, px, py, rb);
	}
	if (__ballot(valid_a || valid_b) == 0ull) return;

	const float4 *rows = reinterpret_cast<const float4 *>(p.row_array);
	uint32_t *stack_a = wave_stack[wave][0], *stack_b = wave_stack[wave][PACKETS - 1];
	*(volatile uint32_t *)&stack_a[0] = kSentinel;
	if (PACKETS == 2) *(volatile uint32_t *)&stack_b[0] = kSentinel;
	PacketRegs A, B;
	rows_init(A, ra, valid_a, (uint32_t)(uintptr_t)(__attribute__((address_space(3))) uint32_t *)(stack_a + 4));
	rows_init(B, rb, valid_b, (uint32_t)(uintptr_t)(__attribute__((address_space(3))) uint32_t *)(stack_b + 4));

	unsigned long long part_a = 0ull, part_b = 0ull;
	const int oct_a = rows_octant(ra, valid_a, part_a);
	const int oct_b = PACKETS == 2 ? rows_octant(rb, valid_b, part_b) : 8;
	uint32_t cnt_n = 0u, cnt_t = 0u;
	uint32_t cnt_w = 0u;
	uint32_t sp_wide = 0u, sp_one = 0u;
	if (p.tile_cost != nullptr && lane == 0u) note_tile_start(p, group_a << 6);
	if (COUNT) *(volatile unsigned long long *)&stack_a[2] = __builtin_amdgcn_s_memtime();
	bool done_a = part_a == 0ull, done_b = part_b == 0ull;
	if (PACKETS == 2 && !done_a && !done_b && oct_a == oct_b && oct_a != 8) {
		*(volatile uint32_t *)&stack_a[4] = kSentinel;
		A.sp += 16u;
		A.mask = part_a; B.mask = part_b;
		if (CULL) {
			const CullRegs cull = cull_setup(ra, rb, valid_a, valid_b, part_a, part_b, p.scene_abs_max, lane);
#define MRT_RWC(O) case O: rows_walk_cull<O, ANY_HIT, COUNT>(rows, p.query_mask, A, B, cull, cnt_n, cnt_t, sp_wide); break;
			switch (oct_a) { MRT_RWC(0) MRT_RWC(1) MRT_RWC(2) MRT_RWC(3) MRT_RWC(4) MRT_RWC(5) MRT_RWC(6) MRT_RWC(7) }
#undef MRT_RWC
		} else {
#define MRT_RW2(O) case O: rows_walk_wide<O, ANY_HIT, COUNT>(rows, p.query_mask, A, B, cnt_n, cnt_t, sp_wide); break;
		switch (oct_a) { MRT_RW2(0) MRT_RW2(1) MRT_RW2(2) MRT_RW2(3) MRT_RW2(4) MRT_RW2(5) MRT_RW2(6) MRT_RW2(7) }
#undef MRT_RW2
		}
		done_a = done_b = true;
	}
#define MRT_RW1(O, S) case O: rows_walk_one<O, ANY_HIT, COUNT>(rows, p.query_mask, S, cnt_n, cnt_t, cnt_w, sp_one); break;
	if (!done_a && oct_a != 8) { switch (oct_a) { MRT_RW1(0, A) MRT_RW1(1, A) MRT_RW1(2, A) MRT_RW1(3, A) MRT_RW1(4, A) MRT_RW1(5, A) MRT_RW1(6, A) MRT_RW1(7, A) } done_a = true; }
	if (PACKETS == 2 && !done_b && oct_b != 8) { switch (oct_b) { MRT_RW1(0, B) MRT_RW1(1, B) MRT_RW1(2, B) MRT_RW1(3, B) MRT_RW1(4, B) MRT_RW1(5, B) MRT_RW1(6, B) MRT_RW1(7, B) } done_b = true; }
#undef MRT_RW1
	uint32_t slot_a = A.bs == 0xFFFFFFFFu ? 0xFFFFFFFFu : A.bs - p.n_nodes, slot_b = B.bs == 0xFFFFFFFFu ? 0xFFFFFFFFu : B.bs - p.n_nodes;
	if (!done_a) {
		uint32_t nn = 0, nt = 0, nd = 0;
		A.bt = ra.t_max;
		packet_traverse<8, ANY_HIT, COUNT>(p, ra, stack_a, A.bt, A.bu, A.bv, slot_a, nn, nt, nd, 0u, 0u, nullptr, !valid_a);
		if (COUNT) { cnt_n += __builtin_amdgcn_readfirstlane(nn); cnt_t += __builtin_amdgcn_readfirstlane(nt); }
		rows_hit_of_slot(rows, p.n_nodes, slot_a, A);
	}
	if (PACKETS == 2 && !done_b) {
		uint32_t nn = 0, nt = 0, nd = 0;
		B.bt = rb.t_max;
		packet_traverse<8, ANY_HIT, COUNT>(p, rb, stack_b, B.bt, B.bu, B.bv, slot_b, nn, nt, nd, 0u, 0u, nullptr, !valid_b);
		if (COUNT) { cnt_n += __builtin_amdgcn_readfirstlane(nn); cnt_t += __builtin_amdgcn_readfirstlane(nt); }
		rows_hit_of_slot(rows, p.n_nodes, slot_b, B);
	}

	{
		const uint32_t lane2 = __builtin_amdgcn_mbcnt_hi(~0u, __builtin_amdgcn_mbcnt_lo(~0u, 0u));
		const uint64_t h_a = ((uint64_t)block_s * (WG / MRT_WAVE) + wave_s) * PACKETS;
		const bool tiled2 = (tile_code >> 16 & 1u) != 0u;
		TileGrid tg2;
		(void)tile_grid(p, tg2);
		const WaveTile ua = {tile_ax, tile_ay, tile_code & 0xFFu}, ub = {tile_bx, tile_by, tile_code >> 8 & 0xFFu};
		uint64_t idx2 = 0; uint32_t px2 = 0, py2 = 0;
		if (tiled2 ? tile_lane(tg2, ua, lane2, idx2, px2, py2) : linear_ray(p, h_a, lane2, idx2, px2, py2))
			finish_row_ray<STREAM>(p, rows, idx2, ra, A.bt, A.bu, A.bv, A.bs, A.bi, slot_a);
		if (PACKETS == 2 && (tiled2 ? tile_lane(tg2, ub, lane2, idx2, px2, py2) : linear_ray(p, h_a + 1u, lane2, idx2, px2, py2)))
			finish_row_ray<STREAM>(p, rows, idx2, rb, B.bt, B.bu, B.bv, B.bs, B.bi, slot_b);
		if (p.tile_cost != nullptr && lane2 == 0u) note_tile_cost(p, h_a << 6);
	}
	const unsigned long long t_start = COUNT ? *(volatile unsigned long long *)&stack_a[2] : 0ull;
	if (COUNT && lane == 0u && (p.count_mode != 2u || (blockIdx.x & 15u) == 0u)) {
		atomicAdd(&p.counters[kCntFetchWaitCycles], (unsigned long long)cnt_w);
		atomicAdd(&p.counters[kCntWaveCycles], __builtin_amdgcn_s_memtime() - t_start);
		atomicAdd(&p.counters[kCntWaves], 1ull);
	}
	if (COUNT && p.count_mode != 2u) {
		const uint32_t base = (uint32_t)(uintptr_t)(__attribute__((address_space(3))) uint32_t *)stack_a;
		const uint32_t e_wide = sp_wide > base ? (sp_wide - base) / 32u : 0u, e_one = sp_one > base ? ((sp_one - base) % 1040u) / 16u : 0u;
		atomicMax(&p.counters[kCntMaxStack], (unsigned long long)(e_wide > e_one ? e_wide : e_one));
	}
	if (COUNT && p.count_mode != 2u) {
		if (valid_a) packet_count(p, cnt_n, cnt_t, 0u, slot_a != 0xFFFFFFFFu, part_a | part_b);
		if (PACKETS == 2 && valid_b) { atomicAdd(&p.counters[kCntRays], 1ull); if (slot_b != 0xFFFFFFFFu) atomicAdd(&p.counters[kCntHits], 1ull); }
	}
}
```

Baseline: 9291.

## Add fast path for packet-rows kernel on aligned 8x8-tiled ray32 grids

Adds a host-side classifier that picks a fast mode when the packet-rows launch uses two packets, 8x8 tiles, ray32 input and hit32 output with no scheduling extras. In that mode the kernel computes tile and lane indices with simple shifts and writes hit records directly after the wide octant walk, skipping the generic tile and linear index math and the finish path. It also derives octants from the precomputed inverse directions, merges pairs of scalar-to-vector moves into 64-bit moves, and zeroes or makes wave-uniform the counters in the walk helpers. The cost is a second specialised code path with alignment conditions that must match the general path exactly.

```diff
diff --git a/__graft_entry__.py b/__graft_entry__.py
--- a/__graft_entry__.py
+++ b/__graft_entry__.py
@@ -26,6 +26,7 @@
     b.build_panorama_data_test()
     b.build_channel_data_test()
     b.build_lane_map_test()
+    b.build_lane_map_fast_test()
     from oracle import pyoracle
     pyoracle.build(force=False)
     if os.path.isdir("/root/reference") and not pyoracle.ref_available():
diff --git a/messyerraytracer_amd/build.py b/messyerraytracer_amd/build.py
--- a/messyerraytracer_amd/build.py
+++ b/messyerraytracer_amd/build.py
@@ -41,6 +41,9 @@
     "lane_map_test": (["host/lane_map_test.cpp"], LANE + ["-O2"], False),
     "lane_map_test_san": (["host/lane_map_test.cpp"], LANE + ["-O1", "-g", "-fno-omit-frame-pointer", "-fsanitize=address,undefined",
                                                               "-fno-sanitize-recover=undefined"], False),
+    "lane_map_fast_test": (["host/lane_map_fast_test.cpp"], LANE + ["-O2"], False),
+    "lane_map_fast_test_san": (["host/lane_map_fast_test.cpp"], LANE + ["-O1", "-g", "-fno-omit-frame-pointer", "-fsanitize=address,undefined",
+                                                                        "-fno-sanitize-recover=undefined"], False),
 }
 
 
@@ -164,6 +167,10 @@
     return build_driver("lane_map_test_san" if sanitize else "lane_map_test", force)
 
 
+def build_lane_map_fast_test(force: bool = False, sanitize: bool = False) -> str:
+    return build_driver("lane_map_fast_test_san" if sanitize else "lane_map_fast_test", force)
+
+
 if __name__ == "__main__":
     print(build_lib(force=True, verbose=True))
     for name in DRIVERS:
diff --git a/messyerraytracer_amd/csrc/kernels.hip b/messyerraytracer_amd/csrc/kernels.hip
--- a/messyerraytracer_amd/csrc/kernels.hip
+++ b/messyerraytracer_amd/csrc/kernels.hip
@@ -75,6 +75,17 @@
 	TraceParams p = p_in;
 	p.tile_group = l.tile_group;
 	const TraceVariant &v = l.v;
+	p.rows_fast = kFastNo;
+	if (v.kernel == TraceKernel::PACKET_ROWS) {
+		FastLaunch f;
+		f.packets = v.packets; f.counting = v.count; f.lane_map = p.lane_map;
+		f.k = p.tile_w_log2; f.order = p.tile_order; f.quarter_all = p.quarter_all;
+		f.sched = p.tile_sched != nullptr; f.perm = p.perm != nullptr; f.tile_cost = p.tile_cost != nullptr;
+		f.ray32_in = p.in_fmt == IN_RAY32; f.hit32_out = p.out_fmt == OUT_HIT32;
+		f.auto_grid = p.auto_grid != nullptr;
+		f.skip = p.skip_flag == nullptr ? 0 : (p.auto_grid != nullptr && p.skip_flag == p.auto_grid + 3 ? 1 : 2);
+		p.rows_fast = fast_launch(f);
+	}
 	const Bool a{v.any_hit}, c{v.count};
 	const auto go = [&](auto kernel) { hipLaunchKernelGGL(kernel, dim3(l.blocks), dim3(l.threads), l.lds, stream, p); };
 	switch (v.kernel) {
diff --git a/messyerraytracer_amd/csrc/lane_map.h b/messyerraytracer_amd/csrc/lane_map.h
--- a/messyerraytracer_amd/csrc/lane_map.h
+++ b/messyerraytracer_amd/csrc/lane_map.h
@@ -155,6 +155,43 @@
 	return true;
 }
 
+struct FastLaunch {
+	uint32_t packets;
+	bool counting;
+	uint32_t lane_map;
+	uint32_t k, order, quarter_all;
+	bool sched, perm, tile_cost;
+	bool ray32_in, hit32_out;
+	bool auto_grid;
+	int skip;
+};
+constexpr uint32_t kFastNo = 0u, kFastOwnGrid = 1u, kFastAutoSkip = 2u, kFastAuto = 3u;
+MRT_LM_HD uint32_t fast_launch(const FastLaunch &f)
+{
+	if (f.packets != 2u || f.counting || f.k != 3u || f.order != 0u || f.quarter_all != 0u) return kFastNo;
+	if (f.sched || f.perm || f.tile_cost || !f.ray32_in || !f.hit32_out) return kFastNo;
+	if (f.lane_map == 1u) return f.skip == 0 ? kFastOwnGrid : kFastNo;
+	if (f.lane_map == 2u && f.auto_grid) return f.skip == 1 ? kFastAutoSkip : (f.skip == 0 ? kFastAuto : kFastNo);
+	return kFastNo;
+}
+MRT_LM_HD bool fast_grid(uint32_t grid_w, uint32_t rows, uint32_t tiles_x)
+{
+	return grid_w != 0u && rows != 0u && (grid_w & 15u) == 0u && (rows & 7u) == 0u && tiles_x == grid_w >> 3 && (((uint64_t)grid_w * rows) >> 32) == 0u;
+}
+MRT_LM_HD bool fast_wave_tile(uint32_t grid_w, uint32_t rows, uint32_t pair, uint32_t &tx, uint32_t &ty)
+{
+	const uint32_t pairs_x = grid_w >> 4;
+	ty = pair / pairs_x;
+	tx = (pair - ty * pairs_x) << 1;
+	return ty < rows >> 3;
+}
+MRT_LM_HD uint32_t fast_tile_ray(uint32_t grid_w, uint32_t tx, uint32_t ty) { return (ty << 3) * grid_w + (tx << 3); }
+MRT_LM_HD uint32_t fast_lane_ray(uint32_t grid_w, uint32_t tile_ray, uint32_t l) { return tile_ray + (l >> 3) * grid_w + (l & 7u); }
+MRT_LM_HD void fast_lane_pixel(uint32_t tx, uint32_t ty, uint32_t l, uint32_t &px, uint32_t &py)
+{
+	px = (tx << 3) + (l & 7u); py = (ty << 3) + (l >> 3);
+}
+
 MRT_LM_HD bool linear_lane(uint64_t group, uint32_t l, uint32_t sparse_lanes, uint64_t count, uint64_t &entry)
 {
 	if (sparse_lanes) { if (l >= sparse_lanes) return false; entry = group * sparse_lanes + l; }
diff --git a/messyerraytracer_amd/csrc/mrt_internal.h b/messyerraytracer_amd/csrc/mrt_internal.h
--- a/messyerraytracer_amd/csrc/mrt_internal.h
+++ b/messyerraytracer_amd/csrc/mrt_internal.h
@@ -114,6 +114,7 @@
 	uint32_t n_nodes;
 	uint32_t count_mode;
 	uint32_t extra_lds;
+	uint32_t rows_fast;
 	mrt_camera cam;
 };
 
diff --git a/messyerraytracer_amd/csrc/packet_rows_kernel.h b/messyerraytracer_amd/csrc/packet_rows_kernel.h
--- a/messyerraytracer_amd/csrc/packet_rows_kernel.h
+++ b/messyerraytracer_amd/csrc/packet_rows_kernel.h
@@ -311,6 +311,23 @@
 	"global_load_dword v60, v55, %[rows]\n"
 #endif
 
+#ifndef MRT_ROWS_PUSH64
+#define MRT_ROWS_PUSH64 1
+#endif
+#if MRT_ROWS_PUSH64
+#define MRT_ROWSW_PUSH_MOVES                                                                                          \
+	"v_mov_b64 v[50:51], s[50:51]\n"                                                                                \
+	"v_mov_b64 v[52:53], s[58:59]\n"                                                                                \
+	"v_mov_b32 v54, s53\n"
+#else
+#define MRT_ROWSW_PUSH_MOVES                                                                                          \
+	"v_mov_b32 v50, s50\n"                                                                                          \
+	"v_mov_b32 v51, s51\n"                                                                                          \
+	"v_mov_b32 v52, s58\n"                                                                                          \
+	"v_mov_b32 v53, s59\n"                                                                                          \
+	"v_mov_b32 v54, s53\n"
+#endif
+
 #define MRT_ROWS_LOOPW(CNT_N, CNT_T, CNT_P, ANYA, ANYB, ANYDONE, BX, BY, BZ)                                                 \
 	asm volatile(                                                                                                   \
 		"s_mov_b64 s[60:61], %[maskA]\n"                                                                            \
@@ -338,11 +355,7 @@
 		"s_cselect_b64 s[58:59], s[42:43], s[40:41]\n"                                                              \
 		"s_cselect_b64 s[60:61], s[36:37], s[38:39]\n"                                        \
 		"s_cselect_b64 s[62:63], s[40:41], s[42:43]\n"                                                              \
-		"v_mov_b32 v50, s50\n"                                                                                      \
-		"v_mov_b32 v51, s51\n"                                                                                      \
-		"v_mov_b32 v52, s58\n"                                                                                      \
-		"v_mov_b32 v53, s59\n"                                                                                      \
-		"v_mov_b32 v54, s53\n"                                                                                      \
+		MRT_ROWSW_PUSH_MOVES                                                                                        \
 		"ds_write_b128 %[spA], v[50:53]\n"                                                                          \
 		"ds_write_b32 %[spA], v54 offset:16\n"                                                                      \
 		"v_add_u32 %[spA], 32, %[spA]\n"                                                                            \
@@ -495,11 +508,7 @@
 		"s_cselect_b64 s[60:61], s[36:37], s[38:39]\n"                                        \
 		"s_cselect_b64 s[62:63], s[40:41], s[42:43]\n"                                                              \
 		"s_cselect_b64 s[66:67], 0, -1\n"                       \
-		"v_mov_b32 v50, s50\n"                                                                                      \
-		"v_mov_b32 v51, s51\n"                                                                                      \
-		"v_mov_b32 v52, s58\n"                                                                                      \
-		"v_mov_b32 v53, s59\n"                                                                                      \
-		"v_mov_b32 v54, s53\n"                                                                                      \
+		MRT_ROWSW_PUSH_MOVES                                                                                        \
 		"ds_write_b128 %[spA], v[50:53]\n"                                                                          \
 		"ds_write_b32 %[spA], v54 offset:16\n"                                                                      \
 		"v_add_u32 %[spA], 32, %[spA]\n"                                                                            \
@@ -581,6 +590,8 @@
 {
 	const float eps = 1e-8f, vneg = -FLT_MAX;
 	uint32_t ev = 0u;
+	if (!COUNT) { cnt_n = 0u; cnt_t = 0u; cnt_w = 0u; sp_max = 0u; }
+	else { cnt_n = __builtin_amdgcn_readfirstlane(cnt_n); cnt_t = __builtin_amdgcn_readfirstlane(cnt_t); cnt_w = __builtin_amdgcn_readfirstlane(cnt_w); sp_max = __builtin_amdgcn_readfirstlane(sp_max); }
 #define MRT_W1(O, BX, BY, BZ)                                                                                         \
 	if (OCT == O) {                                                                                                 \
 		if (COUNT) { if (ANY_HIT) MRT_ROWS_LOOP1(MRT_ROWS_CNT_N, MRT_ROWS_CNT_T, MRT_ROWS_CNT_P, MRT_ROWS_T_PRE, MRT_ROWS_T_POST, MRT_ROWS_ANYHIT("A", "4"), BX, BY, BZ); \
@@ -599,6 +610,8 @@
 __device__ __forceinline__ void rows_walk_wide(const float4 *rows, uint32_t qmask, PacketRegs &a, PacketRegs &b, uint32_t &cnt_n, uint32_t &cnt_t, uint32_t &sp_max)
 {
 	const float eps = 1e-8f, vneg = -FLT_MAX;
+	if (!COUNT) { cnt_n = 0u; cnt_t = 0u; sp_max = 0u; }
+	else { cnt_n = __builtin_amdgcn_readfirstlane(cnt_n); cnt_t = __builtin_amdgcn_readfirstlane(cnt_t); sp_max = __builtin_amdgcn_readfirstlane(sp_max); }
 #define MRT_WW(O, BX, BY, BZ)                                                                                         \
 	if (OCT == O) {                                                                                                 \
 		if (COUNT) { if (ANY_HIT) MRT_ROWS_LOOPW(MRT_ROWS_CNT_N, MRT_ROWS_CNT_T, MRT_ROWS_CNT_P, MRT_ROWSW_ANYHIT("A"), MRT_ROWSW_ANYHIT("B"), MRT_ROWSW_ANYDONE, BX, BY, BZ); \
@@ -617,6 +630,8 @@
 __device__ __forceinline__ void rows_walk_cull(const float4 *rows, uint32_t qmask, PacketRegs &a, PacketRegs &b, const CullRegs &cull, uint32_t &cnt_n, uint32_t &cnt_t, uint32_t &sp_max)
 {
 	const float eps = 1e-8f, vneg = -FLT_MAX;
+	if (!COUNT) { cnt_n = 0u; cnt_t = 0u; sp_max = 0u; }
+	else { cnt_n = __builtin_amdgcn_readfirstlane(cnt_n); cnt_t = __builtin_amdgcn_readfirstlane(cnt_t); sp_max = __builtin_amdgcn_readfirstlane(sp_max); }
 #define MRT_WC(O, BX, BY, BZ)                                                                                         \
 	if (OCT == O) {                                                                                                 \
 		if (COUNT) { if (ANY_HIT) MRT_ROWS_LOOPC(MRT_ROWS_CNT_N, MRT_ROWS_CNT_T, MRT_ROWS_CNT_P, MRT_ROWSW_ANYHIT("A"), MRT_ROWSW_ANYHIT("B"), MRT_ROWSW_ANYDONE, BX, BY, BZ); \
@@ -693,11 +708,10 @@
 	s.sp = sp; s.cur = 0u; s.mask = 0ull;
 }
 
-__device__ __forceinline__ int rows_octant(const RayRegs &r, bool part, unsigned long long &part_mask)
+__device__ __forceinline__ int rows_octant(const PacketRegs &s, bool part, unsigned long long &part_mask)
 {
 	part_mask = __ballot(part);
-	const unsigned long long sx = __ballot(part && safe_inv(r.dx) < 0.0f), sy = __ballot(part && safe_inv(r.dy) < 0.0f),
-			sz = __ballot(part && safe_inv(r.dz) < 0.0f);
+	const unsigned long long sx = __ballot(part && s.ix < 0.0f), sy = __ballot(part && s.iy < 0.0f), sz = __ballot(part && s.iz < 0.0f);
 	const bool uniform = (sx == 0ull || sx == part_mask) && (sy == 0ull || sy == part_mask) && (sz == 0ull || sz == part_mask);
 	return uniform ? ((sx ? 1 : 0) | (sy ? 2 : 0) | (sz ? 4 : 0)) : 8;
 }
@@ -726,6 +740,59 @@
 	store_hit<STREAM>(p, ray_idx, r, best_t, prim, best_u, best_v, nx, ny, nz, layers, best_slot);
 }
 
+template <bool STREAM>
+__device__ __forceinline__ void load_ray32(const float4 *q, RayRegs &r)
+{
+	const float4 a = STREAM ? stream_load4(q) : q[0], b = STREAM ? stream_load4(q + 1) : q[1];
+	r.ox = a.x; r.oy = a.y; r.oz = a.z; r.t_max = a.w;
+	r.dx = b.x; r.dy = b.y; r.dz = b.z; r.t_min = b.w;
+}
+__device__ __forceinline__ void row_record32(const float4 *rows, float best_t, float best_u, float best_v, uint32_t best_row, uint32_t best_id, float4 &a, float4 &b)
+{
+	a.x = best_t; a.y = __int_as_float(-1); a.z = best_u; a.w = best_v;
+	b.x = 0.0f; b.y = 0.0f; b.z = 0.0f; b.w = __uint_as_float(0u);
+	if (best_row != 0xFFFFFFFFu) {
+		const float4 *row = rows + (size_t)best_row * 4u;
+		a.y = __uint_as_float(best_id);
+		const float4 nn = row[3];
+		b.x = nn.x; b.y = nn.y; b.z = nn.z;
+		b.w = reinterpret_cast<const float *>(row)[7];
+	}
+}
+struct RowsWave;
+template <bool STREAM> __device__ __forceinline__ void rows_fast_records(const RowsWave &w, const PacketRegs &A, const PacketRegs &B);
+__device__ __forceinline__ const __attribute__((address_space(4))) TraceParams *rows_args_again()
+{
+	const __attribute__((address_space(4))) TraceParams *q =
+			(const __attribute__((address_space(4))) TraceParams *)__builtin_amdgcn_kernarg_segment_ptr();
+	asm volatile("" : "+s"(q));
+	return q;
+}
+
+struct RowsWave {
+	uint32_t block_s, wave_s, tile_ax, tile_ay, tile_bx, tile_by, tile_code;
+	uint32_t fast_ray, fast_w;
+};
+typedef __attribute__((address_space(3))) uint32_t *RowsStack;
+static_assert((kAutoGridOff * sizeof(unsigned long long)) % 16u == 0u && (kDetectScratchOff - kAutoGridOff) * sizeof(unsigned long long) >= 16u,
+		"the grid words of detect_grid_kernel: 16-byte aligned, four of them");
+template <bool STREAM>
+__device__ __forceinline__ void rows_fast_records(const RowsWave &w, const PacketRegs &A, const PacketRegs &B)
+{
+	const TraceParams &p2 = *(const TraceParams *)rows_args_again();
+	const uint32_t lane2 = __builtin_amdgcn_mbcnt_hi(~0u, __builtin_amdgcn_mbcnt_lo(~0u, 0u));
+	float4 *out = reinterpret_cast<float4 *>(p2.hits) + (size_t)fast_lane_ray(w.fast_w, w.fast_ray, lane2) * 2u;
+	const float4 *rows2 = reinterpret_cast<const float4 *>(p2.row_array);
+	float4 aa, ab, ba, bb;
+	row_record32(rows2, A.bt, A.bu, A.bv, A.bs, A.bi, aa, ab);
+	row_record32(rows2, B.bt, B.bu, B.bv, B.bs, B.bi, ba, bb);
+	if (STREAM) { stream_store4(out, aa); stream_store4(out + 1, ab); stream_store4(out + 16, ba); stream_store4(out + 17, bb); }
+	else { out[0] = aa; out[1] = ab; out[16] = ba; out[17] = bb; }
+}
+template <bool ANY_HIT, bool COUNT, int PACKETS, int WG, bool CULL, bool FAST>
+__device__ __forceinline__ bool rows_walks_and_records(const TraceParams &p, RowsStack lds_a, RowsStack lds_b, uint32_t lane,
+		RayRegs &ra, RayRegs &rb, bool valid_a, bool valid_b, const RowsWave &w);
+
 #ifndef MRT_ROWS_WPE
 #define MRT_ROWS_WPE 8
 #endif
@@ -733,7 +800,6 @@
 __global__ __launch_bounds__(WG) __attribute__((amdgpu_waves_per_eu(MRT_ROWS_WPE, 8))) void trace_packet_rows_kernel(const TraceParams p)
 {
 	__shared__ __attribute__((aligned(16))) uint32_t wave_stack[WG / MRT_WAVE][PACKETS][(MRT_PACKET_STACK + 1) * 4];
-	if (skip_launch(p)) return;
 	constexpr bool STREAM = WG == MRT_WAVE;
 	uint32_t block = blockIdx.x;
 	if (p.xcd_swizzle) {
@@ -742,47 +808,82 @@
 	}
 	const uint32_t wave = threadIdx.x / MRT_WAVE, lane = threadIdx.x & (MRT_WAVE - 1);
 	const uint32_t wave_s = __builtin_amdgcn_readfirstlane(wave), block_s = block;
-	const uint64_t group_a = ((uint64_t)block_s * (WG / MRT_WAVE) + wave_s) * PACKETS;
-	TileGrid tg;
-	const bool tiled = tile_grid(p, tg);
-	WaveTile ta = {0u, 0u, kPieceNone}, tb = ta;
-	if (tiled) {
-		ta = wave_tile(tg, group_a);
-		if (PACKETS == 2) tb = wave_tile_next(tg, ta, group_a);
-	}
-	const uint32_t tile_ax = __builtin_amdgcn_readfirstlane(ta.tx), tile_ay = __builtin_amdgcn_readfirstlane(ta.ty);
-	const uint32_t tile_bx = __builtin_amdgcn_readfirstlane(tb.tx), tile_by = __builtin_amdgcn_readfirstlane(tb.ty);
-	const uint32_t tile_code = __builtin_amdgcn_readfirstlane((ta.code & 0xFFu) | (tb.code & 0xFFu) << 8 | (tiled ? 1u << 16 : 0u));
-	uint64_t idx = 0; uint32_t px = 0, py = 0;
-	const bool valid_a = tiled ? tile_lane(tg, ta, lane, idx, px, py) : linear_ray(p, group_a, lane, idx, px, py);
 	RayRegs ra = {0.0f, 0.0f, 0.0f, 0.0f, 0.0f, 0.0f, 1.0f, 0.0f}, rb = ra;
-	if (valid_a) load_ray<STREAM>(p, idx, px, py, ra);
-	bool valid_b = false;
-	if (PACKETS == 2) {
-		valid_b = tiled ? tile_lane(tg, tb, lane, idx, px, py) : linear_ray(p, group_a + 1u, lane, idx, px, py);
-		if (valid_b) load_ray<STREAM>(p, idx, px, py, rb);
-	}
-	if (__ballot(valid_a || valid_b) == 0ull) return;
-
+	bool valid_a = false, valid_b = false;
+	uint32_t tile_ax = 0u, tile_ay = 0u, tile_bx = 0u, tile_by = 0u, tile_code = 0u;
+	if (PACKETS == 2 && !COUNT && p.rows_fast != kFastNo) {
+		const uint32_t how = p.rows_fast;
+		uint32_t gw = p.grid_w, n_rows = p.rows, tiles_x = p.tiles_x;
+		if (how != kFastOwnGrid) {
+			const uint4 found = *reinterpret_cast<const uint4 *>(p.auto_grid);
+			if ((how == kFastAutoSkip) & (found.w == p.skip_when)) return;
+			gw = found.x; n_rows = found.y; tiles_x = found.z;
+		}
+		if (fast_grid(gw, n_rows, tiles_x)) {
+			uint32_t tx = 0u, ty = 0u;
+			if (!fast_wave_tile(gw, n_rows, block_s * (WG / MRT_WAVE) + wave_s, tx, ty)) return;
+			const RowsWave w = {0u, 0u, 0u, 0u, 0u, 0u, 0u, fast_tile_ray(gw, tx, ty), gw};
+			const float4 *q = reinterpret_cast<const float4 *>(p.rays) + (size_t)fast_lane_ray(gw, w.fast_ray, lane) * 2u;
+			load_ray32<STREAM>(q, ra);
+			load_ray32<STREAM>(q + 16, rb);
+			if (rows_walks_and_records<ANY_HIT, COUNT, PACKETS, WG, CULL, true>(p, (RowsStack)wave_stack[wave_s][0], (RowsStack)wave_stack[wave_s][PACKETS - 1], lane, ra, rb, true, true, w))
+				return;
+			valid_a = valid_b = true;
+			tile_ax = tx; tile_ay = ty; tile_bx = tx + 1u; tile_by = ty; tile_code = kPieceTile | kPieceTile << 8 | 1u << 16;
+		}
+	}
+	const TraceParams &pg = *(const TraceParams *)rows_args_again();
+	if (tile_code == 0u) {
+		if (skip_launch(pg)) return;
+		const uint64_t group_a = ((uint64_t)block_s * (WG / MRT_WAVE) + wave_s) * PACKETS;
+		TileGrid tg;
+		const bool tiled = tile_grid(pg, tg);
+		WaveTile ta = {0u, 0u, kPieceNone}, tb = ta;
+		if (tiled) {
+			ta = wave_tile(tg, group_a);
+			if (PACKETS == 2) tb = wave_tile_next(tg, ta, group_a);
+		}
+		tile_ax = __builtin_amdgcn_readfirstlane(ta.tx); tile_ay = __builtin_amdgcn_readfirstlane(ta.ty);
+		tile_bx = __builtin_amdgcn_readfirstlane(tb.tx); tile_by = __builtin_amdgcn_readfirstlane(tb.ty);
+		tile_code = __builtin_amdgcn_readfirstlane((ta.code & 0xFFu) | (tb.code & 0xFFu) << 8 | (tiled ? 1u << 16 : 0u));
+		uint64_t idx = 0; uint32_t px = 0, py = 0;
+		valid_a = tiled ? tile_lane(tg, ta, lane, idx, px, py) : linear_ray(pg, group_a, lane, idx, px, py);
+		if (valid_a) load_ray<STREAM>(pg, idx, px, py, ra);
+		if (PACKETS == 2) {
+			valid_b = tiled ? tile_lane(tg, tb, lane, idx, px, py) : linear_ray(pg, group_a + 1u, lane, idx, px, py);
+			if (valid_b) load_ray<STREAM>(pg, idx, px, py, rb);
+		}
+		if (__ballot(valid_a || valid_b) == 0ull) return;
+		if (pg.tile_cost != nullptr && lane == 0u) note_tile_start(pg, group_a << 6);
+	}
+	const RowsWave w = {block_s, wave_s, tile_ax, tile_ay, tile_bx, tile_by, tile_code, 0u, 0u};
+	rows_walks_and_records<ANY_HIT, COUNT, PACKETS, WG, CULL, false>(pg, (RowsStack)wave_stack[wave][0], (RowsStack)wave_stack[wave][PACKETS - 1], lane, ra, rb, valid_a, valid_b, w);
+}
+
+template <bool ANY_HIT, bool COUNT, int PACKETS, int WG, bool CULL, bool FAST>
+__device__ __forceinline__ bool rows_walks_and_records(const TraceParams &p, RowsStack lds_a, RowsStack lds_b, uint32_t lane,
+		RayRegs &ra, RayRegs &rb, bool valid_a, bool valid_b, const RowsWave &w)
+{
+	constexpr bool STREAM = WG == MRT_WAVE;
+	uint32_t *stack_a = (uint32_t *)lds_a, *stack_b = (uint32_t *)lds_b;
+	const uint32_t block_s = w.block_s, wave_s = w.wave_s, tile_ax = w.tile_ax, tile_ay = w.tile_ay, tile_bx = w.tile_bx, tile_by = w.tile_by, tile_code = w.tile_code;
 	const float4 *rows = reinterpret_cast<const float4 *>(p.row_array);
-	uint32_t *stack_a = wave_stack[wave][0], *stack_b = wave_stack[wave][PACKETS - 1];
-	*(volatile uint32_t *)&stack_a[0] = kSentinel;
-	if (PACKETS == 2) *(volatile uint32_t *)&stack_b[0] = kSentinel;
+	*(volatile __attribute__((address_space(3))) uint32_t *)&lds_a[0] = kSentinel;
+	if (PACKETS == 2) *(volatile __attribute__((address_space(3))) uint32_t *)&lds_b[0] = kSentinel;
 	PacketRegs A, B;
-	rows_init(A, ra, valid_a, (uint32_t)(uintptr_t)(__attribute__((address_space(3))) uint32_t *)(stack_a + 4));
-	rows_init(B, rb, valid_b, (uint32_t)(uintptr_t)(__attribute__((address_space(3))) uint32_t *)(stack_b + 4));
+	rows_init(A, ra, valid_a, (uint32_t)(uintptr_t)(lds_a + 4));
+	rows_init(B, rb, valid_b, (uint32_t)(uintptr_t)(lds_b + 4));
 
 	unsigned long long part_a = 0ull, part_b = 0ull;
-	const int oct_a = rows_octant(ra, valid_a, part_a);
-	const int oct_b = PACKETS == 2 ? rows_octant(rb, valid_b, part_b) : 8;
+	const int oct_a = rows_octant(A, valid_a, part_a);
+	const int oct_b = PACKETS == 2 ? rows_octant(B, valid_b, part_b) : 8;
 	uint32_t cnt_n = 0u, cnt_t = 0u;
 	uint32_t cnt_w = 0u;
 	uint32_t sp_wide = 0u, sp_one = 0u;
-	if (p.tile_cost != nullptr && lane == 0u) note_tile_start(p, group_a << 6);
-	if (COUNT) *(volatile unsigned long long *)&stack_a[2] = __builtin_amdgcn_s_memtime();
+	if (COUNT) *(volatile __attribute__((address_space(3))) unsigned long long *)&lds_a[2] = __builtin_amdgcn_s_memtime();
 	bool done_a = part_a == 0ull, done_b = part_b == 0ull;
 	if (PACKETS == 2 && !done_a && !done_b && oct_a == oct_b && oct_a != 8) {
-		*(volatile uint32_t *)&stack_a[4] = kSentinel;
+		*(volatile __attribute__((address_space(3))) uint32_t *)&lds_a[4] = kSentinel;
 		A.sp += 16u;
 		A.mask = part_a; B.mask = part_b;
 		if (CULL) {
@@ -796,25 +897,28 @@
 #undef MRT_RW2
 		}
 		done_a = done_b = true;
-	}
+		if (FAST) { rows_fast_records<STREAM>(w, A, B); return true; }
+	}
+	if (FAST) return false;
 #define MRT_RW1(O, S) case O: rows_walk_one<O, ANY_HIT, COUNT>(rows, p.query_mask, S, cnt_n, cnt_t, cnt_w, sp_one); break;
 	if (!done_a && oct_a != 8) { switch (oct_a) { MRT_RW1(0, A) MRT_RW1(1, A) MRT_RW1(2, A) MRT_RW1(3, A) MRT_RW1(4, A) MRT_RW1(5, A) MRT_RW1(6, A) MRT_RW1(7, A) } done_a = true; }
 	if (PACKETS == 2 && !done_b && oct_b != 8) { switch (oct_b) { MRT_RW1(0, B) MRT_RW1(1, B) MRT_RW1(2, B) MRT_RW1(3, B) MRT_RW1(4, B) MRT_RW1(5, B) MRT_RW1(6, B) MRT_RW1(7, B) } done_b = true; }
 #undef MRT_RW1
-	uint32_t slot_a = A.bs == 0xFFFFFFFFu ? 0xFFFFFFFFu : A.bs - p.n_nodes, slot_b = B.bs == 0xFFFFFFFFu ? 0xFFFFFFFFu : B.bs - p.n_nodes;
+	const TraceParams &p2 = p;
+	uint32_t slot_a = A.bs == 0xFFFFFFFFu ? 0xFFFFFFFFu : A.bs - p2.n_nodes, slot_b = B.bs == 0xFFFFFFFFu ? 0xFFFFFFFFu : B.bs - p2.n_nodes;
 	if (!done_a) {
 		uint32_t nn = 0, nt = 0, nd = 0;
 		A.bt = ra.t_max;
-		packet_traverse<8, ANY_HIT, COUNT>(p, ra, stack_a, A.bt, A.bu, A.bv, slot_a, nn, nt, nd, 0u, 0u, nullptr, !valid_a);
+		packet_traverse<8, ANY_HIT, COUNT>(p2, ra, stack_a, A.bt, A.bu, A.bv, slot_a, nn, nt, nd, 0u, 0u, nullptr, !valid_a);
 		if (COUNT) { cnt_n += __builtin_amdgcn_readfirstlane(nn); cnt_t += __builtin_amdgcn_readfirstlane(nt); }
-		rows_hit_of_slot(rows, p.n_nodes, slot_a, A);
+		rows_hit_of_slot(rows, p2.n_nodes, slot_a, A);
 	}
 	if (PACKETS == 2 && !done_b) {
 		uint32_t nn = 0, nt = 0, nd = 0;
 		B.bt = rb.t_max;
-		packet_traverse<8, ANY_HIT, COUNT>(p, rb, stack_b, B.bt, B.bu, B.bv, slot_b, nn, nt, nd, 0u, 0u, nullptr, !valid_b);
+		packet_traverse<8, ANY_HIT, COUNT>(p2, rb, stack_b, B.bt, B.bu, B.bv, slot_b, nn, nt, nd, 0u, 0u, nullptr, !valid_b);
 		if (COUNT) { cnt_n += __builtin_amdgcn_readfirstlane(nn); cnt_t += __builtin_amdgcn_readfirstlane(nt); }
-		rows_hit_of_slot(rows, p.n_nodes, slot_b, B);
+		rows_hit_of_slot(rows, p2.n_nodes, slot_b, B);
 	}
 
 	{
@@ -822,28 +926,29 @@
 		const uint64_t h_a = ((uint64_t)block_s * (WG / MRT_WAVE) + wave_s) * PACKETS;
 		const bool tiled2 = (tile_code >> 16 & 1u) != 0u;
 		TileGrid tg2;
-		(void)tile_grid(p, tg2);
+		(void)tile_grid(p2, tg2);
 		const WaveTile ua = {tile_ax, tile_ay, tile_code & 0xFFu}, ub = {tile_bx, tile_by, tile_code >> 8 & 0xFFu};
 		uint64_t idx2 = 0; uint32_t px2 = 0, py2 = 0;
-		if (tiled2 ? tile_lane(tg2, ua, lane2, idx2, px2, py2) : linear_ray(p, h_a, lane2, idx2, px2, py2))
-			finish_row_ray<STREAM>(p, rows, idx2, ra, A.bt, A.bu, A.bv, A.bs, A.bi, slot_a);
-		if (PACKETS == 2 && (tiled2 ? tile_lane(tg2, ub, lane2, idx2, px2, py2) : linear_ray(p, h_a + 1u, lane2, idx2, px2, py2)))
-			finish_row_ray<STREAM>(p, rows, idx2, rb, B.bt, B.bu, B.bv, B.bs, B.bi, slot_b);
-		if (p.tile_cost != nullptr && lane2 == 0u) note_tile_cost(p, h_a << 6);
-	}
-	const unsigned long long t_start = COUNT ? *(volatile unsigned long long *)&stack_a[2] : 0ull;
-	if (COUNT && lane == 0u && (p.count_mode != 2u || (blockIdx.x & 15u) == 0u)) {
-		atomicAdd(&p.counters[kCntFetchWaitCycles], (unsigned long long)cnt_w);
-		atomicAdd(&p.counters[kCntWaveCycles], __builtin_amdgcn_s_memtime() - t_start);
-		atomicAdd(&p.counters[kCntWaves], 1ull);
-	}
-	if (COUNT && p.count_mode != 2u) {
-		const uint32_t base = (uint32_t)(uintptr_t)(__attribute__((address_space(3))) uint32_t *)stack_a;
+		if (tiled2 ? tile_lane(tg2, ua, lane2, idx2, px2, py2) : linear_ray(p2, h_a, lane2, idx2, px2, py2))
+			finish_row_ray<STREAM>(p2, rows, idx2, ra, A.bt, A.bu, A.bv, A.bs, A.bi, slot_a);
+		if (PACKETS == 2 && (tiled2 ? tile_lane(tg2, ub, lane2, idx2, px2, py2) : linear_ray(p2, h_a + 1u, lane2, idx2, px2, py2)))
+			finish_row_ray<STREAM>(p2, rows, idx2, rb, B.bt, B.bu, B.bv, B.bs, B.bi, slot_b);
+		if (p2.tile_cost != nullptr && lane2 == 0u) note_tile_cost(p2, h_a << 6);
+	}
+	const unsigned long long t_start = COUNT ? *(volatile __attribute__((address_space(3))) unsigned long long *)&lds_a[2] : 0ull;
+	if (COUNT && lane == 0u && (p2.count_mode != 2u || (blockIdx.x & 15u) == 0u)) {
+		atomicAdd(&p2.counters[kCntFetchWaitCycles], (unsigned long long)cnt_w);
+		atomicAdd(&p2.counters[kCntWaveCycles], __builtin_amdgcn_s_memtime() - t_start);
+		atomicAdd(&p2.counters[kCntWaves], 1ull);
+	}
+	if (COUNT && p2.count_mode != 2u) {
+		const uint32_t base = (uint32_t)(uintptr_t)lds_a;
 		const uint32_t e_wide = sp_wide > base ? (sp_wide - base) / 32u : 0u, e_one = sp_one > base ? ((sp_one - base) % 1040u) / 16u : 0u;
-		atomicMax(&p.counters[kCntMaxStack], (unsigned long long)(e_wide > e_one ? e_wide : e_one));
-	}
-	if (COUNT && p.count_mode != 2u) {
-		if (valid_a) packet_count(p, cnt_n, cnt_t, 0u, slot_a != 0xFFFFFFFFu, part_a | part_b);
-		if (PACKETS == 2 && valid_b) { atomicAdd(&p.counters[kCntRays], 1ull); if (slot_b != 0xFFFFFFFFu) atomicAdd(&p.counters[kCntHits], 1ull); }
-	}
-}
+		atomicMax(&p2.counters[kCntMaxStack], (unsigned long long)(e_wide > e_one ? e_wide : e_one));
+	}
+	if (COUNT && p2.count_mode != 2u) {
+		if (valid_a) packet_count(p2, cnt_n, cnt_t, 0u, slot_a != 0xFFFFFFFFu, part_a | part_b);
+		if (PACKETS == 2 && valid_b) { atomicAdd(&p2.counters[kCntRays], 1ull); if (slot_b != 0xFFFFFFFFu) atomicAdd(&p2.counters[kCntHits], 1ull); }
+	}
+	return true;
+}
```

New measurement: 9824, median of 6. 5.7% higher.
